# duckmayr/gpirt

Measured on AMD Instinct MI355X. Metric: MCMC iterations/sec at N=8192 x m=1024, higher is better.
Workload: dtype f64

## Files before the change

gpirt_amd/_lib.py:

```python
from __future__ import annotations

import ctypes as C
import os

import numpy as np

HERE = os.path.dirname(os.path.abspath(__file__))
LIB_PATH = os.environ.get("GPIRT_HIP_LIBRARY") or os.path.join(HERE, "libgpirt_hip.so")

NGRID = 1001
RNG_RSTREAM, RNG_ITEM = 0, 1
ST_INIT_F, ST_INIT_BETA, ST_F_Z, ST_F_ESS, ST_FSTAR, ST_THETA, ST_BETA = 1, 2, 3, 4, 5, 6, 7
ST_PPC = 8
ST_ELL = 9
ST_AMP = 10
ST_CARRY = 11

E_ARG, E_HIP, E_NODEVICE, E_ALLOC, E_RNG, E_INTERRUPT, E_NUMERIC = -1, -2, -3, -4, -5, -6, -7

SUM_THETA_BETA, SUM_F, SUM_PRED, SUM_WAIC = 1, 2, 4, 8
SUM_PARTS = {"theta_beta": SUM_THETA_BETA, "f": SUM_F, "pred": SUM_PRED, "waic": SUM_WAIC}
SUM_DIAG = 16
SUM_THETA_HIST, SUM_IRF_BAND = 32, 128
SUM_PARTS.update(diag=SUM_DIAG, theta_hist=SUM_THETA_HIST, irf_band=SUM_IRF_BAND)
# ... 670 lines not shown
    "gpirt_sampler_shape_order_state": (_i32, [_vp, C.POINTER(_vp), C.POINTER(_i64)]),
    "gpirt_shape_order_state_bytes": (_i32, [_i64, _i32, C.POINTER(_i64)]),
    "gpirt_shape_order_combine": (_i32, [_vp, _i32, C.POINTER(_vp), C.POINTER(ShapeOrder)]),
    "gpirt_sampler_summary_accumulate": (_i32, [_vp]),
    "gpirt_sampler_summary_get": (_i32, [_vp, C.c_char_p, _dp, _i64]),
    "gpirt_sampler_summary_totals": (_i32, [_vp, _dp]),
    "gpirt_sampler_create": (_i32, [C.POINTER(_vp), _vp, _dp, _i64, _i64, _dp, _dp, _dp, _dp,
                                     C.POINTER(Options), _vp]),
    "gpirt_sampler_destroy": (_i32, [_vp]),
    "gpirt_sampler_init": (_i32, [_vp]),
    "gpirt_sampler_step": (_i32, [_vp]),
    "gpirt_sampler_draw_f": (_i32, [_vp]),
    "gpirt_sampler_draw_fstar": (_i32, [_vp]),
    "gpirt_sampler_theta_partial": (_i32, [_vp]),
    "gpirt_sampler_theta_finish": (_i32, [_vp]),
    "gpirt_sampler_set_theta_block": (_i32, [_vp, _vp, _i64, _i64, _i64]),
    "gpirt_sampler_theta_block": (_i32, [_vp]),
    "gpirt_sampler_theta_commit": (_i32, [_vp]),
    "gpirt_sampler_draw_beta": (_i32, [_vp]),
    "gpirt_sampler_factor": (_i32, [_vp]),
    "gpirt_sampler_skip_factor": (_i32, [_vp]),
    "gpirt_sampler_adopt_factor": (_i32, [_vp, _i32]),
    "gpirt_sampler_build_cov": (_i32, [_vp]),
    "gpirt_sampler_panel_factor": (_i32, [_vp, _i64]),
    "gpirt_sampler_panel_update": (_i32, [_vp, _i64, _i64]),
    "gpirt_sampler_panel_copy": (_i32, [_vp, _i64, _vp, _i32]),
    "gpirt_sampler_panel_rows": (_i32, [_vp, C.POINTER(_i64)]),
    "gpirt_sampler_panel_factor_part": (_i32, [_vp, _i64, _i32]),
    "gpirt_sampler_panel_update_part": (_i32, [_vp, _i64, _i64, _i32]),
    "gpirt_sampler_panel_copy_part": (_i32, [_vp, _i64, _i32, _vp, _i64, _i32]),
    "gpirt_sampler_ldl": (_i32, [_vp, C.POINTER(_i64)]),
    "gpirt_sampler_nu_lr_draws": (_i32, [_vp, C.POINTER(_i64)]),
    "gpirt_sampler_ess_pack_draws": (_i32, [_vp, C.POINTER(_i64)]),
    "gpirt_sampler_nu_lr_rows": (_i32, [_vp, _vp, _i64]),
    "gpirt_sampler_fstar_free_draws": (_i32, [_vp, C.POINTER(_i64)]),
    "gpirt_sampler_factor_lr_count": (_i32, [_vp, C.POINTER(_i64)]),
    "gpirt_sampler_dense_factor_count": (_i32, [_vp, C.POINTER(_i64)]),
    "gpirt_sampler_dense_factor": (_i32, [_vp]),
    "gpirt_sampler_factor_lr_parts": (_i32, [_vp, _vp, _i64]),
    "gpirt_sampler_factor_lr_width": (_i32, [_vp, C.POINTER(_i32)]),
    "gpirt_sampler_factor_lr_blocks": (_i32, [_vp, _vp, _i64]),
    "gpirt_sampler_copy_state": (_i32, [_vp, _vp]),
    "gpirt_sampler_accumulate_irf": (_i32, [_vp]),
    "gpirt_sampler_iteration": (_i32, [_vp, C.POINTER(_i32)]),
    "gpirt_sampler_check": (_i32, [_vp]),
    "gpirt_sampler_devptr": (_i32, [_vp, C.c_char_p, C.POINTER(_vp), C.POINTER(_i64)]),
    "gpirt_sampler_get": (_i32, [_vp, C.c_char_p, _vp, _i64]),
    "gpirt_sampler_set": (_i32, [_vp, C.c_char_p, _dp, _i64]),
    "gpirt_sampler_finish_irfs": (_i32, [_vp, _i32, _dp]),
    "gpirt_sampler_enable_timing": (_i32, [_vp, _i32]),
    "gpirt_sampler_stage_times": (_i32, [_vp, _dp, _i32, C.POINTER(_i32), C.POINTER(C.c_char_p)]),
    "gpirt_prof_trailing": (_i32, [_vp, _i32, _dp, C.POINTER(_i64), _dp]),
    "gpirt_prof_enable": (_i32, [_vp, _i32]),
    "gpirt_prof_syrk": (_i32, [_vp, _i32, _i32, _dp, C.POINTER(_i64), _dp]),
    "gpirt_prof_syrk_bytes": (_i32, [_vp, _i32, _dp]),
    "gpirt_sampler_set_iteration": (_i32, [_vp, _i32]),
    "gpirt_ell_grid": (_i32, [_dbl, _dbl, _i32, _dp]),
    "gpirt_ell_check": (_i32, [_dbl, _dbl, _i32, _dp, _i32, _i32, C.POINTER(Kernel), C.POINTER(Options), _i64]),
    "gpirt_sampler_ell_enable": (_i32, [_vp, _dbl, _dbl, _i32, _dp, _i32, _i32, _i32]),
    "gpirt_sampler_draw_ell": (_i32, [_vp]),
    "gpirt_sampler_ell_width": (_i32, [_vp, _i32]),
    "gpirt_sampler_ell_get": (_i32, [_vp, C.c_char_p, _vp, _i64]),
    "gpirt_sampler_ell_stats": (_i32, [_vp, C.POINTER(Ell)]),
    "gpirt_sampler_draw_ell_centred": (_i32, [_vp]),
    "gpirt_sampler_ell_width_centred": (_i32, [_vp, _i32]),
    "gpirt_sampler_ell_centred_stats": (_i32, [_vp, C.POINTER(EllCentred)]),
# ... 109 lines not shown
```

gpirt_amd/csrc/api.hip:

```cpp
#include "common.h"
#include "kernels.h"
#include "rstream.h"

#include <stdarg.h>
#include <stdlib.h>
#include <new>
#include <vector>
#include <algorithm>

namespace gpirt {

static thread_local char g_err[512] = "";

static int env_value(const char* name, int dflt)
{
    const char* v = getenv(name);
    if (!v || !*v) return dflt;
    return atoi(v);
}
const Config& env_config()
{
    static const Config c = [] {
        Config d;
        d.nbo = env_value("GPIRT_NBO", d.nbo);            d.nbp = env_value("GPIRT_NBP", d.nbp);
        d.lookahead = env_value("GPIRT_LOOKAHEAD", d.lookahead);
        d.panel = env_value("GPIRT_PANEL", d.panel);      d.defer = env_value("GPIRT_DEFER", d.defer);
        d.trsm_inv = env_value("GPIRT_TRSM_INV", d.trsm_inv);
        d.ll_exact = env_value("GPIRT_LL_EXACT", d.ll_exact);
        d.ess_screen = env_value("GPIRT_ESS_SCREEN", d.ess_screen);
        d.theta_fixed = env_value("GPIRT_THETA_FIXED", d.theta_fixed);
        d.bordered = env_value("GPIRT_BORDERED", d.bordered);
        d.early_inv = env_value("GPIRT_EARLY_INV", d.early_inv);
        d.prep_early = env_value("GPIRT_PREP_EARLY", d.prep_early);
        d.guard_verbose = env_value("GPIRT_GUARD_VERBOSE", d.guard_verbose);
        d.rs_predict = env_value("GPIRT_RS_PREDICT", d.rs_predict);
        d.rs_lr = env_value("GPIRT_RS_LR", d.rs_lr);
        d.nu_lr = env_value("GPIRT_NU_LR", d.nu_lr);
        d.nu_sub = env_value("GPIRT_NU_SUB", NU_LR_SUB);
        d.fstar_free = env_value("GPIRT_FSTAR_FREE", d.fstar_free);
        d.factor_lr = env_value("GPIRT_FACTOR_LR", d.factor_lr);
        d.flr_fuse = env_value("GPIRT_FLR_FUSE", d.flr_fuse);
        d.flr_narrow = env_value("GPIRT_FLR_NARROW", d.flr_narrow);
        d.beta_screen = env_value("GPIRT_BETA_SCREEN", d.beta_screen);
        d.zfill_compact = env_value("GPIRT_ZFILL_COMPACT", d.zfill_compact);
        d.ess_pack = env_value("GPIRT_ESS_PACK", d.ess_pack);
        if (d.nbo < 64) d.nbo = 1024;
        if (d.nbp != 0 && d.nbp < 64) d.nbp = 512;
        return d;
    }();
    return c;
}

void set_error(const char* fmt, ...)
{
    va_list ap;
    va_start(ap, fmt);
    vsnprintf(g_err, sizeof(g_err), fmt, ap);
    va_end(ap);
}

int ensure_work(gpirt_handle_t h, size_t bytes)
{
    if (bytes <= h->work_bytes) return 0;
    GP_HIP(hipStreamSynchronize(h->stream));
    if (h->d_work) GP_HIP(hipFree(h->d_work));
    h->d_work = nullptr;
    h->work_bytes = 0;
    hipError_t e = hipMalloc(&h->d_work, bytes);
    if (e != hipSuccess) { set_error("hipMalloc(%zu) failed: %s", bytes, hipGetErrorString(e)); return GPIRT_E_ALLOC; }
    h->work_bytes = bytes;
    GP_HIP(poison_fresh(h, h->d_work, bytes, h->stream));
    return 0;
}

static int check_device(int device)
{
    int count = 0;
    hipError_t e = hipGetDeviceCount(&count);
// ... 55 lines not shown
}

}

using namespace gpirt;

static int create_own_stream(gpirt_handle_t* out, int device, bool high_priority);
namespace gpirt {
int create_side_handle(gpirt_handle_t* out, int device) { return create_own_stream(out, device, true); }
}

namespace gpirt {
int prof_pair_begin(gpirt_handle_t h, hipStream_t stream, ProfPair& pp)
{
    pp = ProfPair{nullptr, nullptr, 0.0, 0, 0.0};
    if (!h->prof.enabled) return 0;
    if (!h->prof.free_pairs.empty()) { pp = h->prof.free_pairs.back(); h->prof.free_pairs.pop_back(); }
    else { GP_HIP(hipEventCreate(&pp.e0)); GP_HIP(hipEventCreate(&pp.e1)); }
    GP_HIP(hipEventRecord(pp.e0, stream));
    return 0;
}
int prof_pair_end(gpirt_handle_t h, hipStream_t stream, ProfPair& pp, int cls, double flops, double bytes)
{
    if (!pp.e0) return 0;
    GP_HIP(hipEventRecord(pp.e1, stream));
    pp.flops = flops; pp.bytes = bytes; pp.cls = cls;
    h->prof.pending.push_back(pp);
    return 0;
}
}

extern "C" {

int gpirt_version(void) { return 143; }

const char* gpirt_last_error(void) { return g_err; }

int gpirt_device_count(int* count)
{
    GP_ARG(count != nullptr);
    int c = 0;
    hipError_t e = hipGetDeviceCount(&c);
    *count = (e == hipSuccess) ? c : 0;
    return 0;
}

int gpirt_create(gpirt_handle_t* out, int device, void* stream)
{
    GP_ARG(out != nullptr);
    *out = nullptr;
    GP_TRY(check_device(device < 0 ? 0 : device));
    if (device >= 0) GP_HIP(hipSetDevice(device));
    int cur = 0;
    GP_HIP(hipGetDevice(&cur));
    hipDeviceProp_t prop;
    GP_HIP(hipGetDeviceProperties(&prop, cur));
    if (strncmp(prop.gcnArchName, "gfx950", 6) != 0) {
        set_error("device %d is %s; libgpirt_hip is built for gfx950 (MI355X) only", cur, prop.gcnArchName);
        return GPIRT_E_NODEVICE;
    }
    gpirt_handle_s* h = new (std::nothrow) gpirt_handle_s();
    if (!h) { set_error("out of host memory"); return GPIRT_E_ALLOC; }
    h->device = cur;
    h->cfg = env_config();
    h->n_cu = prop.multiProcessorCount;
    h->stream = (hipStream_t)stream;
    h->own_stream = false;
// ... 63 lines not shown
    hipError_t e = hipSuccess;
    if (high_priority) e = hipDeviceGetStreamPriorityRange(&lo_pri, &hi_pri);
    if (e == hipSuccess)
        e = high_priority ? hipStreamCreateWithPriority(&st, hipStreamNonBlocking, hi_pri)
                          : hipStreamCreateWithFlags(&st, hipStreamNonBlocking);
    if (e != hipSuccess) { set_error("hipStreamCreate failed: %s", hipGetErrorString(e)); return GPIRT_E_HIP; }
    const int rc = gpirt_create(out, device, st);
    if (rc != 0) { hipStreamDestroy(st); return rc; }
    (*out)->own_stream = true;
    return 0;
}

int gpirt_create_own_stream(gpirt_handle_t* out, int device) { return create_own_stream(out, device, false); }

static int* config_slot(gpirt_handle_t h, const char* name, bool* read_only)
{
    struct E { const char* k; int* p; bool ro; } tab[] = {
        { "GPIRT_NBO", &h->cfg.nbo, true }, { "GPIRT_NBP", &h->cfg.nbp, true },
        { "GPIRT_LOOKAHEAD", &h->cfg.lookahead, false }, { "GPIRT_PANEL", &h->cfg.panel, false },
        { "GPIRT_DEFER", &h->cfg.defer, false }, { "GPIRT_TRSM_INV", &h->cfg.trsm_inv, false },
        { "GPIRT_LL_EXACT", &h->cfg.ll_exact, false }, { "GPIRT_ESS_SCREEN", &h->cfg.ess_screen, false }, { "GPIRT_THETA_FIXED", &h->cfg.theta_fixed, false }, { "GPIRT_BORDERED", &h->cfg.bordered, false },
        { "GPIRT_EARLY_INV", &h->cfg.early_inv, false }, { "GPIRT_PREP_EARLY", &h->cfg.prep_early, false },
        { "GPIRT_RS_PREDICT", &h->cfg.rs_predict, false },
        { "GPIRT_RS_LR", &h->cfg.rs_lr, false },
        { "GPIRT_NU_LR", &h->cfg.nu_lr, false },
        { "GPIRT_NU_SUB", &h->cfg.nu_sub, false },
        { "GPIRT_FSTAR_FREE", &h->cfg.fstar_free, false },
        { "GPIRT_FACTOR_LR", &h->cfg.factor_lr, false },
        { "GPIRT_FLR_FUSE", &h->cfg.flr_fuse, false },
        { "GPIRT_FLR_NARROW", &h->cfg.flr_narrow, false },
        { "GPIRT_BETA_SCREEN", &h->cfg.beta_screen, false },
        { "GPIRT_ZFILL_COMPACT", &h->cfg.zfill_compact, false },
        { "GPIRT_ESS_PACK", &h->cfg.ess_pack, false },
    };
    for (auto& e : tab)
        if (strcmp(e.k, name) == 0) { if (read_only) *read_only = e.ro; return e.p; }
    return nullptr;
}

int gpirt_config_get(gpirt_handle_t h, const char* name, int* value)
{
    GP_ARG(h && name && value);
    int* p = config_slot(h, name, nullptr);
    if (!p) { set_error("unknown switch '%s'", name); return GPIRT_E_ARG; }
    *value = *p;
    return 0;
}

int gpirt_config_set(gpirt_handle_t h, const char* name, int value)
{
    GP_ARG(h && name);
    bool ro = false;
    int* p = config_slot(h, name, &ro);
    if (!p) { set_error("unknown switch '%s'", name); return GPIRT_E_ARG; }
    if (ro) { set_error("%s is fixed per process (set it in the environment before the library is loaded)", name); return GPIRT_E_ARG; }
    if (p == &h->cfg.nu_sub && !nu_lr_sub_ok(value)) { set_error("GPIRT_NU_SUB must be 64, 128, 256 or 512 (got %d)", value); return GPIRT_E_ARG; }
    GP_HIP(hipStreamSynchronize(h->stream));
    *p = value;
    if (h->aux) *config_slot(h->aux, name, nullptr) = value;
    return 0;
}

void gpirt_kernel_default(gpirt_kernel* k)
{
    if (!k) return;
    memset(k, 0, sizeof(*k));
// ... 475 lines not shown
{
    GP_ARG(h && d_beta && d_theta && d_y && d_f && d_pm && d_ps && d_step && n >= 0 && m >= 0);
    BetaArgs a{};
    a.beta = d_beta; a.theta = d_theta; a.y = d_y; a.f = d_f; a.pm = d_pm; a.ps = d_ps; a.step = d_step;
    a.n = n; a.m = m; a.N = GPIRT_NGRID; a.mu = nullptr; a.mu_star = nullptr;
    a.seed = seed; a.iter = iter; a.item0 = 0; a.U = nullptr; a.path = d_path;
    if (h->cfg.beta_screen == 1 && n <= 8192 && n * m > 0) {
        GP_TRY(ensure_work(h, 8 * sizeof(double)));
        int* bad = reinterpret_cast<int*>(h->d_work);
        GP_HIP(hipMemsetAsync(bad, 0, sizeof(int), h->stream));
        GP_TRY(launch_check_y(h->stream, d_y, n * m, bad));
        GP_HIP(hipMemcpyAsync(h->h_info, bad, sizeof(int), hipMemcpyDeviceToHost, h->stream));
        GP_HIP(hipStreamSynchronize(h->stream));
        a.screen = *h->h_info == 0;
    }
    return launch_draw_beta(h->stream, a);
}

int gpirt_draw_beta(gpirt_handle_t h, double* d_beta, const double* d_theta, const double* d_y,
                    const double* d_f, const double* d_pm, const double* d_ps, const double* d_step,
                    int64_t n, int64_t m, uint64_t seed, uint32_t iter)
{
    return draw_beta_op(h, d_beta, d_theta, d_y, d_f, d_pm, d_ps, d_step, n, m, seed, iter, nullptr);
}

int gpirt_draw_beta_paths(gpirt_handle_t h, double* d_beta, const double* d_theta, const double* d_y,
                          const double* d_f, const double* d_pm, const double* d_ps, const double* d_step,
                          int64_t n, int64_t m, uint64_t seed, uint32_t iter, int* d_path)
{
    GP_ARG(d_path != nullptr);
    return draw_beta_op(h, d_beta, d_theta, d_y, d_f, d_pm, d_ps, d_step, n, m, seed, iter, d_path);
}

int gpirt_prof_enable(gpirt_handle_t h, int on)
{
    GP_ARG(h != nullptr);
    h->prof.enabled = on != 0;
    return 0;
}

static int prof_resolve(gpirt_handle_t h)
{
    if (h->prof.pending.empty()) return 0;
    GP_HIP(hipStreamSynchronize(h->stream));
    if (h->side) GP_HIP(hipStreamSynchronize(h->side));
    float longest4 = 0.f;
    {
        std::vector<float> d4;
        for (auto& pp : h->prof.pending)
            if (pp.cls == 4) { float ms = 0.f; GP_HIP(hipEventElapsedTime(&ms, pp.e0, pp.e1)); d4.push_back(ms); }
        if (!d4.empty()) { std::sort(d4.begin(), d4.end()); longest4 = d4[(d4.size() * 3) / 4]; }
    }
    for (auto& pp : h->prof.pending) {
        float ms = 0.f;
        GP_HIP(hipEventElapsedTime(&ms, pp.e0, pp.e1));
        if (pp.cls == 4 && ms < 0.25f * longest4) { h->prof.free_pairs.push_back(pp); continue; }
        h->prof.ms[pp.cls] += ms;
        h->prof.launches[pp.cls] += 1;
        h->prof.flops[pp.cls] += pp.flops;
        h->prof.bytes[pp.cls] += pp.bytes;
        h->prof.free_pairs.push_back(pp);
    }
    h->prof.pending.clear();
    return 0;
}

// ... 104 lines not shown
```

gpirt_amd/csrc/common.h:

```cpp
#pragma once

#include <hip/hip_runtime.h>
#include <stdint.h>
#include <stdio.h>
#include <string.h>
#include <math.h>
#include <vector>

#include "../../include/gpirt_hip.h"

namespace gpirt {

void set_error(const char* fmt, ...);

#define GP_HIP(call)                                                                         \
    do {                                                                                     \
        hipError_t e_ = (call);                                                              \
        if (e_ != hipSuccess) {                                                              \
            gpirt::set_error("%s failed: %s (%s:%d)", #call, hipGetErrorString(e_), __FILE__, \
                             __LINE__);                                                      \
            return GPIRT_E_HIP;                                                              \
        }                                                                                    \
    } while (0)

// ... 14 lines not shown
constexpr int PROF_CLASSES = 6;
struct ProfPair { hipEvent_t e0, e1; double flops; int cls; double bytes; };
struct Prof {
    bool        enabled = false;
    double      ms[PROF_CLASSES] = {};
    int64_t     launches[PROF_CLASSES] = {};
    double      flops[PROF_CLASSES] = {};
    double      bytes[PROF_CLASSES] = {};
    std::vector<ProfPair> pending;
    std::vector<ProfPair> free_pairs;
};

struct Config {
    int  nbo = 1024, nbp = 0;
    int  lookahead = 1;
    int  panel = 1;
    int  defer = 0;
    int  trsm_inv = 1;
    int  ll_exact = 0;
    int  theta_fixed = 1;
    int  ess_screen = 1;
    int  bordered = 1;
    int  early_inv = 1;
    int  prep_early = 1;
    int  rs_lr = 1;
    int  nu_lr = 1;
    int  nu_sub = 0;
    int  fstar_free = 1;
    int  factor_lr = 1;
    int  flr_fuse = 1;
    int  flr_narrow = 1;
    int  beta_screen = 1;
    int  ess_pack = 1;
    int  zfill_compact = 1;
    int  rs_predict = 1;
    int  guard_verbose = 0;
};
const Config& env_config();

struct KernelSpec {
    int    family = GPIRT_KERNEL_SE;
    double length_scale = 1.0;
    double inv_ell = 1.0;
    bool is_default() const { return family == GPIRT_KERNEL_SE && length_scale == 1.0; }
};

}

struct gpirt_handle_s {
    int          device = 0;
    gpirt::Config cfg;
    gpirt::KernelSpec kern;
    hipStream_t  stream = nullptr;
    bool         own_stream = false;
    int*         d_info = nullptr;
    int*         h_info = nullptr;
    double*      d_work = nullptr;
    size_t       work_bytes = 0;
    gpirt::Prof  prof;
    hipStream_t  side = nullptr;
    hipEvent_t   ev_fork = nullptr, ev_join = nullptr, ev_mid = nullptr, ev_half = nullptr;
    gpirt_handle_t aux = nullptr;
    const double* inv_partial_L = nullptr;
    int64_t      inv_partial_pairs = 0;
    bool         slim_leaf = false;
    hipEvent_t   ev_prelast = nullptr;
// ... 161 lines not shown
```

gpirt_amd/csrc/kernels.h:

```cpp
#pragma once

#include "common.h"

namespace gpirt {

enum { TRI_NONE = 0, TRI_SYRK_LOWER = 1, TRI_A_LOWER = 2, TRI_A_UPPER = 3, TRI_SYRK_LOWER_TRAILING = 4,
       TRI_SYRK_LOWER_BACKGROUND = 5  };
bool gemm_trailing_uses_128(int64_t M, int64_t N, bool background = false);
int launch_gemm_update_potf2(hipStream_t stream, int64_t M, int64_t N, int64_t K, const double* P, int64_t ldp,
                             double* C, int64_t ldc, int nb_next, int k0_next, int* info);

int launch_gemm(gpirt_handle_t h, hipStream_t stream, bool ta, bool tb, int tri, int64_t M,
                int64_t N, int64_t K, double alpha, const double* A, int64_t lda, const double* B,
                int64_t ldb, double beta, double* C, int64_t ldc, int64_t Mread = 0, const int* run_if = nullptr);

int launch_gemm_batched(hipStream_t stream, bool ta, bool tb, int tri, int64_t M, int64_t N, int64_t K, double alpha,
                        const double* A, int64_t lda, int64_t strideA, const double* B, int64_t ldb, int64_t strideB,
                        double beta, double* C, int64_t ldc, int64_t strideC, int batch);
int launch_gemm_batched_dual(hipStream_t stream, int tri, int64_t M, int64_t N, int64_t K, const double* A, int64_t lda,
                             int64_t strideA, const double* B, int64_t ldb, int64_t strideB, int64_t K2, const double* A2,
                             int64_t lda2, int64_t strideA2, const double* B2, int64_t ldb2, int64_t strideB2, double* C,
                             int64_t ldc, int64_t strideC, int batch);

int launch_syrk_panels(hipStream_t stream, int64_t M, int64_t N, int64_t kpart, int nparts, double alpha, const double* A,
// ... 380 lines not shown
struct TfDims { int64_t mp, ksteps, iblocks, gblocks; };
TfDims tf_dims(int64_t n, int64_t m, int64_t N);
size_t tf_y8_bytes(const TfDims& d);
size_t tf_gq_bytes(const TfDims& d);
size_t tf_aux_bytes(const TfDims& d);
int* tf_overflow(void* aux, const TfDims& d);
int launch_tf_indicators(hipStream_t stream, const double* y, int64_t n, int64_t ldy, int64_t m, const TfDims& d, void* Y8);
int launch_theta_fixed(hipStream_t stream, const double* fstar, int64_t N, int64_t n, int64_t m, const TfDims& d,
                       const void* Y8, void* Gq, void* aux, double* logpost, int64_t ldlp, bool trace = false,
                       gpirt_handle_t prof = nullptr);
long long* tf_trace(void* aux, const TfDims& d);
int tf_trace_wgs();
struct ThetaArgs {
    const double* logpost;
    int64_t N, n;
    int64_t i0;
    int stabilise;
    uint64_t seed; uint32_t iter;
    const double* U; uint64_t* pos; uint64_t cap;
    double* theta_out; int* degenerate; int* err;
    const double* log_prior; const int32_t* codes;
};
int launch_theta_sample(hipStream_t stream, const ThetaArgs& a);

struct BetaArgs {
    double* beta; const double* theta; const double* y; const double* f;
    const double* pm; const double* ps; const double* step;
    int64_t n, m, N;
    double* mu; double* mu_star;
    uint64_t seed; uint32_t iter; uint32_t item0;
    const double* U; uint64_t* pos; const uint64_t* item_off; uint64_t cap; int* err;
    int screen;
    int* path;
};
int launch_draw_beta(hipStream_t stream, const BetaArgs& a);
int launch_linear_mean(hipStream_t stream, const double* x, int64_t n, const double* beta, int64_t m, double* mu);

int prof_pair_begin(gpirt_handle_t h, hipStream_t stream, ProfPair& pp);
int prof_pair_end(gpirt_handle_t h, hipStream_t stream, ProfPair& pp, int cls, double flops, double bytes);

int report_panel_guard(gpirt_handle_t h, const int* info_words, hipStream_t stream);

int create_side_handle(gpirt_handle_t* out, int device);

constexpr int SUM_LAYOUT_VERSION = 1;
constexpr int SUM_HEADER_WORDS = 8;
struct SumLayout {
    int64_t tb_mean = -1, tb_m2 = -1, lse = -1, ll_mean = -1, ll_m2 = -1, y = -1, p_sum = -1, f_mean = -1, f_m2 = -1, irf = -1;
    int64_t dtb[7] = { -1, -1, -1, -1, -1, -1, -1 };
    int64_t df[7] = { -1, -1, -1, -1, -1, -1, -1 };
    int64_t total = 0;
};
enum { DG_H1_MEAN, DG_H1_M2, DG_H2_MEAN, DG_H2_M2, DG_BSUM, DG_BM_MEAN, DG_BM_M2 };
SumLayout summary_layout(int64_t n, int64_t m, int parts);
struct QntLayout {
    int64_t th_hist[3] = { -1, -1, -1 };
    int64_t th_off = -1;
    int64_t psum = -1;
    int64_t band_nan = -1;
    int64_t band = -1;
    int64_t total = 0;
};
QntLayout quantile_layout(int64_t n, int64_t m, int parts);
void irf_band_edges(double* out);
struct SummaryState {
    int parts = 0;
    int64_t n = 0, m = 0, draws = 0, planned = 0;
    double* block = nullptr;
// ... 521 lines not shown
```

gpirt_amd/csrc/sampler.hip:

```cpp
#include "common.h"
#include "kernels.h"
#include "rstream.h"

#include <stdlib.h>
#include <new>
#include <mutex>
#include <type_traits>
#include <string>
#include <vector>

using namespace gpirt;

namespace {

constexpr int KSPLIT = 16;

enum { ST_DRAW_F = 0, ST_FSTAR, ST_THETA_GEMM, ST_THETA_SAMPLE, ST_BETA, ST_FACTOR, ST_COUNT };
const char* const kStageNames[ST_COUNT] = { "draw_f", "draw_fstar", "theta_gemm", "theta_sample",
                                            "draw_beta", "factor" };

}

enum { ELL_WHITENED = 0, ELL_CENTRED = 1 };
struct EllUpdate {
// ... 88 lines not shown
    BetaCentredArgs a{};
    int prior_ok = -1;
    hipEvent_t tev[4] = {};
    double last_ms = 0.0, item_ms = 0.0;
};

struct ScaleState {
    bool on = false;
    uint32_t t[2] = {};
    double width[2] = {};
    ScaleArgs a{};
    int last_kind = -1;
    int prior_ok = -1;
    hipEvent_t tev[7] = {};
    double last_ms[2] = {};
    double times[6] = {};
};

struct CarryState {
    int64_t calls = 0;
    unsigned long long* counters = nullptr;
    double* quad = nullptr;
    hipEvent_t tev[2] = {};
    double last_ms = 0.0;
};

struct gpirt_sampler_s {
    gpirt_handle_t h = nullptr;
    int64_t n = 0, m = 0, N = GPIRT_NGRID;
    gpirt_options opt{};
    KernelSpec kern;
    RStream* rs = nullptr;
    double *y = nullptr, *Ypm = nullptr, *theta = nullptr, *theta_new = nullptr, *f = nullptr,
           *Z = nullptr, *NU = nullptr, *beta = nullptr, *mu = nullptr, *mu_star = nullptr,
           *fstar = nullptr, *L = nullptr, *tstar = nullptr, *kstar = nullptr, *rhs = nullptr,
           *mean = nullptr, *s = nullptr, *Gpm = nullptr, *logpost = nullptr, *irf_sum = nullptr,
           *pm = nullptr, *ps = nullptr, *step = nullptr;
    int kr = 0;
    double *knodes = nullptr, *kV = nullptr, *kparts = nullptr, *kP = nullptr;
    int64_t ext = 0, ldl = 0, node_off = -1, rank_off = 0;
    bool ext_grid = false, rows_valid = false, fstar_rows = false;
    double *nu_nodes = nullptr, *nu_wts = nullptr, *nuV = nullptr, *nuT = nullptr;
    bool nu_kern_ok = false, theta_ok = false, theta_alone = false;
    int64_t nu_lr_draws = 0;
    gpirt_handle_t haux = nullptr;
    hipEvent_t ev_trmm = nullptr, ev_prep = nullptr;
    bool prep_valid = false, prep_pending = false;
    double *ffF = nullptr, *ffW = nullptr;
    bool ff_have = false, prep_free = false;
    double ff_ell = 0.0;
    int64_t fstar_free_draws = 0;
    double *theta_L = nullptr, *flrG = nullptr, *flrXh = nullptr, *flrX = nullptr, *flrD = nullptr;
    bool L_structured = false;
    int L_part_width = 0;
    hipEvent_t ev_flr = nullptr;
    int64_t factor_lr_count = 0, dense_factor_count = 0;
    uint32_t z_filled_iter = 0;
    hipEvent_t ev_zfill = nullptr;
    bool beta_deferred = false, beta_pending = false;
    hipEvent_t ev_beta = nullptr;
    int64_t blk_i0 = 0, blk_n = 0, blk_m = 0;
    double *Ypm_blk = nullptr, *Gpm_full = nullptr, *logpost_blk = nullptr, *fstar_full = nullptr, *theta_stage = nullptr;
    TfDims tfd{}, tfd_blk{};
    double *tf_y8 = nullptr, *tf_gq = nullptr, *tf_aux = nullptr, *tf_y8_blk = nullptr, *tf_gq_blk = nullptr, *tf_aux_blk = nullptr;
    int *ess_k = nullptr, *flags = nullptr;
    int *fstar_off = nullptr;
    int *h_flags = nullptr;
// ... 31 lines not shown
    bool initialised = false;
    bool sticky_info = false;
    bool factor_fresh = false;
    bool counted = false;
    bool in_init = false;
    bool timing = false;
    hipEvent_t ev[ST_COUNT + 1] = {};
    double stage_ms[ST_COUNT] = {};
    std::vector<void*> allocs;
    std::vector<double> host_tmp;
    SummaryState sum;
    PpcState ppc;
    RankState rank;
    ShapeState shape;
    ScoreState score;
    SumscoreState sumscore;
    EquateState equate;
    LooState loo;
    AcfState acf;
    GroupsState groups;
    EllState ell;
    AmpState amp;
    OrdState ord;
    PopState pop;
    CarryState carry;
    SmoothF sf;
    BetaCentredState bc;
    ScaleState sc;
    bool lp_current = false;
    bool mu_linear = false;
    uint32_t* ess_ypk = nullptr;
    bool ess_ypk_valid = false;
    int64_t ess_pack_draws = 0;
};

namespace {

template <typename T>
int dalloc(gpirt_sampler_s* s, T** p, size_t count, bool numbers = true)
{
    void* q = nullptr;
    const size_t bytes = (count ? count : 1) * sizeof(T);
    hipError_t e = hipMalloc(&q, bytes);
    if (e != hipSuccess) {
        set_error("hipMalloc(%zu bytes) failed: %s", bytes, hipGetErrorString(e));
        return GPIRT_E_ALLOC;
    }
    s->allocs.push_back(q);
    *p = reinterpret_cast<T*>(q);
    if (std::is_same<T, double>::value || std::is_same<T, float>::value) {
        if (numbers && poison_fresh(s->h, q, bytes, s->h->stream) != hipSuccess) {
            set_error("hipMemsetAsync(%zu bytes) failed", bytes);
            return GPIRT_E_HIP;
        }
    }
    return 0;
}

inline bool stream_mode(const gpirt_sampler_s* s) { return s->opt.rng_kind == GPIRT_RNG_RSTREAM; }

int report_degenerate_theta(gpirt_sampler_s* s, int count);

void ahead_generate(gpirt_sampler_s* s, uint32_t* dst, uint64_t count)
{
    constexpr uint64_t EVERY = 1ull << 16;
    while (count) {
        const uint64_t c = count < EVERY ? count : EVERY;
        s->snaps.emplace_back(s->ahead_gen, *s->rs);
        s->rs->fill_raw(dst, c);
        s->ahead_gen += c; dst += c; count -= c;
    }
}

void ahead_resolve(void* owner, bool gone)
{
    gpirt_sampler_s* s = static_cast<gpirt_sampler_s*>(owner);
    if (s->ahead_attached) {
        if (s->ev_up) hipEventSynchronize(s->ev_up);
        size_t best = 0;
        for (size_t q = 0; q < s->snaps.size(); ++q) if (s->snaps[q].first <= s->ahead_used) best = q;
        *s->rs = s->snaps[best].second;
        s->rs->skip(s->ahead_used - s->snaps[best].first);
    }
    s->ahead_attached = false;
    s->snaps.clear();
    s->ahead_gen = s->ahead_used = s->a_len = 0;
    if (s->rs_obj) { s->rs_obj->owner = nullptr; s->rs_obj->resolve = nullptr; }
    if (gone) { s->rs_obj = nullptr; s->rs = nullptr; }
}

void rstream_forget(void* sampler)
{
// ... 223 lines not shown
        if (nu_lr && s->prep_pending && s->prep_free) {
            GP_HIP(hipStreamWaitEvent(st, s->ev_prep, 0));
            s->prep_pending = false;
        }
        if (s->z_filled_iter == iter && s->ev_zfill) {
            GP_HIP(hipStreamWaitEvent(st, s->ev_zfill, 0));
            s->z_filled_iter = 0;
        } else {
            GP_TRY(z_sync(s));
            GP_TRY(launch_item_uniforms(st, s->opt.seed, iter, GPIRT_ST_F_Z, (uint32_t)s->opt.item0, m, n, s->Z, true, s->h->cfg.zfill_compact == 1));
        }
        {
            ProfPair pp;
            GP_TRY(prof_pair_begin(h, st, pp));
            if (nu_lr) {
                double flops = 0.0, bytes = 0.0;
                NuLrArgs q{};
                q.L = s->L; q.ldl = s->ldl; q.Bt = s->L + n + s->node_off; q.V = s->nuV; q.Z = s->Z; q.NU = s->NU; q.T = s->nuT;
                q.n = n; q.m = m; q.sub = h->cfg.nu_sub;
                GP_TRY(launch_nu_lr_basis(st, s->theta, n, s->nu_nodes, s->nu_wts, s->nuV));
                if (free) GP_HIP(hipEventRecord(s->ev_trmm, st));
                GP_TRY(launch_nu_lr(st, q, &flops, &bytes));
                GP_TRY(prof_pair_end(h, st, pp, 3, flops, bytes));
                s->nu_lr_draws += 1;
            } else {
                GP_TRY(launch_gemm(h, st, false, false, TRI_A_LOWER, n, m, n, 1.0, s->L, s->ldl, s->Z, n, 0.0, s->NU, n));
                GP_TRY(prof_pair_end(h, st, pp, 3, (double)n * (double)n * (double)m, 8.0 * (0.5 * (double)n * (double)n + 2.0 * (double)n * (double)m)));
            }
        }
        if (s->amp.mode) GP_TRY(launch_amp_scale(st, s->NU, s->amp.amp, n, m));
        if (prep && !early && !free) GP_HIP(hipEventRecord(s->ev_trmm, st));
        if (s->ord.on) {
            EssOrdArgs a{};
            a.f = s->f; a.nu = s->NU; a.mu = s->mu; a.cat = s->ord.cat; a.thr = s->ord.thr; a.counts = s->ord.counts;
            a.C = s->ord.C; a.n = n; a.m = m; a.k_out = s->ess_k; a.err = s->flags;
            a.seed = s->opt.seed; a.iter = iter; a.item0 = (uint32_t)s->opt.item0;
            a.screen = h->cfg.ess_screen == 1;
            GP_TRY(launch_ess_ord(st, a));
        } else {
        EssArgs a{};
        a.f = s->f; a.nu = s->NU; a.y = s->y; a.mu = s->mu; a.n = n; a.m = m; a.k_out = s->ess_k;
        a.err = s->flags; a.seed = s->opt.seed; a.iter = iter; a.item0 = (uint32_t)s->opt.item0;
        a.ll_exact = h->cfg.ll_exact;
        a.screen = h->cfg.ess_screen == 1;
        if (h->cfg.ess_pack != 2 && s->mu_linear && s->ess_ypk && !s->opt.kernel_fp32 && ess_pack_eligible(n)) {
            if (!s->ess_ypk_valid) { GP_TRY(launch_ess_pack(st, s->y, n, m, s->ess_ypk)); s->ess_ypk_valid = true; }
            a.ypk = s->ess_ypk; a.theta = s->theta; a.beta = s->beta;
            a.grid = h->cfg.ess_pack == 3 ? 2 * h->n_cu : 0;
            s->ess_pack_draws += 1;
        }
        GP_TRY(launch_ess(st, a));
        }
        if (prep) {
            hipStream_t ax = s->haux->stream;
            GP_HIP(hipStreamWaitEvent(ax, s->ev_trmm, 0));
            if (free) {
                GP_TRY(fstar_prep_free(s, ax, !nu_lr));
            } else {
                s->haux->slim_leaf = early;
                const int rc_prep = fstar_prep(s, s->haux);
                s->haux->slim_leaf = false;
                GP_TRY(rc_prep);
            }
            GP_HIP(hipEventRecord(s->ev_prep, ax));
            s->prep_valid = true; s->prep_pending = true; s->prep_free = free;
        }
        return 0;
    }
    auto plain_item = [&](int64_t j) -> int {
        GP_TRY(launch_rstream_normals(st, s->U, s->pos, 0, n, 1, s->Z));
        GP_TRY(launch_trmv_lower(st, s->L, n, s->ldl, s->Z, s->NU + n, s->NU));
        EssArgs a{};
        a.f = s->f + j * n; a.nu = s->NU; a.y = s->y + j * n; a.mu = s->mu + j * n; a.n = n; a.m = 1;
        a.k_out = s->ess_k + j; a.err = s->flags; a.item0 = (uint32_t)j;
        a.U = s->U; a.pos = s->pos; a.cap = s->U_cap;
        return launch_ess(st, a);
    };
    const bool spec = s->spec_ok;
    if (!spec) {
        for (int64_t j = 0; j < m; ++j) GP_TRY(plain_item(j));
        return 0;
    }
    bool tiles64 = false;
    Rs3Args a{};
    a.U = s->U; a.cap = s->U_cap; a.Nrm = s->Nrm; a.anchor = s->anchor; a.pos = s->pos; a.posv = s->posv; a.k_out = s->ess_k;
    a.err = s->flags; a.n = n; a.m = m; a.Lt = s->Lt; a.nkb = rs_tile_quads(n); a.part = s->rs_part;
    a.units = s->rs_units; a.nunits = s->rs_nunits; a.nfull = s->rs_nfull;
    a.lim1 = RS3_C1; a.lim2 = RS3_C2;
    if (h->rs_cand_limit > 0) {
        if (h->rs_cand_limit < a.lim1) a.lim1 = h->rs_cand_limit;
        if (h->rs_cand_limit < a.lim2) a.lim2 = h->rs_cand_limit;
    }
    a.f = s->f; a.y = s->y; a.mu = s->mu; a.partial = s->rs_partial; a.flags = s->rs_flags;
    GP_TRY(launch_rs3_begin(st, a, (uint64_t)m * (2ull * (uint64_t)n + 2ull) + 512ull * (uint64_t)m + 4096ull));
    int64_t pass = 0, done = 0;
    int64_t one_phase = 0;
    bool topped = false;
    bool predict = h->cfg.rs_predict != 2;
    bool lr = predict && s->lr_on, lr_missed = false;
    bool tiles32_full = !lr;
    if (predict) GP_TRY(launch_rs32_tiles(st, s->L, n, s->ldl, s->Lt32, lr));
    if (lr) {
        RsLrSetup q{};
        q.theta = s->theta; q.n = n; q.nodes = s->lr_nodes; q.wts = s->lr_wts; q.Mn = s->lr_M; q.eps = GPIRT_JITTER; q.L = s->L; q.ldl = s->ldl;
        q.V64 = s->lr_V64; q.Gb = s->lr_Gb; q.V32t = s->lr_V32t; q.Ct32 = s->lr_Ct32; q.nk8 = rs32_tile_octs(n); q.bad = s->lr_bad;
        GP_TRY(launch_rs_lr_setup(st, q));
    }
    while (done < m) {
        const int64_t left = m - done;
        int64_t count = (left + RS3_SLOTS - 1) / RS3_SLOTS + left / 40 + 2;
        if (one_phase > 4 * m + 64) { set_error("R-stream replay: draw_f made no progress"); return GPIRT_E_NUMERIC; }
        if (predict) {
            count = (left + RS3_SLOTS - 1) / RS3_SLOTS + left / 8 + 4;
            if (s->rs_pass_rate > 0.0) {
                const int64_t hint = (int64_t)(s->rs_pass_rate * 1.03 * (double)left) + 4;
                if (hint < count) count = hint;
            }
            Rs3Args ap = a;
            ap.anchor = s->anchorP; ap.pos = s->rs_posP; ap.k_out = s->rs_kpred; ap.err = s->rs_errP;
            ap.units = s->rs_unitsP; ap.nunits = s->rs_nunitsP; ap.nfull = s->rs_nfullP;
            if (!lr && !tiles32_full) { GP_TRY(launch_rs32_tiles(st, s->L, n, s->ldl, s->Lt32)); tiles32_full = true; }
            ap.lr = lr ? 1 : 0;
            if (lr) {
                ap.units = s->lr_units; ap.nunits = ap.nfull = s->lr_nunits;
                ap.Ct32 = s->lr_Ct32; ap.lrY = s->lr_Y; ap.V32t = s->lr_V32t;
            }
            ap.Lt32 = s->Lt32; ap.nk8 = rs32_tile_octs(n); ap.part32 = s->rs_part32; ap.mispredict = h->rs_mispredict;
            ap.dec_part = s->rs_dec_part; ap.dec_rec = s->rs_dec_rec; ap.dec_ticket = s->rs_dec_ticket; ap.pass_count = s->rs_ctl + 3;
            GP_TRY(launch_rs_pred_start(st, s->anchor, s->anchorP, s->ess_k, m));
            for (int64_t q = 0; q < count; ++q, ++pass) {
                s->rs_tag += 1ull << 20;
                ap.tag = s->rs_tag;
                ap.trace = (h->rs_trace_pass >= 0 && pass == h->rs_trace_pass) ? s->rs_trace : nullptr;
                ProfPair pp;
                GP_TRY(prof_pair_begin(h, st, pp));
                GP_TRY(launch_rs3p_products(st, ap));
                const double pass_el = lr ? (double)(RS3P_KC + RS_LR_RANK) * (double)n : 0.5 * (double)n * (double)(n + 1);
                GP_TRY(prof_pair_end(h, st, pp, 4, 2.0 * RS3_CAND * pass_el, 4.0 * pass_el));
                if (lr) GP_TRY(launch_rs_lr_apply(st, ap));
                GP_TRY(launch_rs3p_decide(st, ap));
            }
            const int64_t mc = m - done;
            GP_TRY(launch_rs_gather(st, s->Nrm, s->posv, s->anchorP, n, done, m, s->Z));
            GP_TRY(launch_gemm(h, st, false, false, TRI_A_LOWER, n, mc, n, 1.0, s->L, s->ldl, s->Z, n, 0.0, s->NU, n));
            RsVerifyArgs v{};
            v.f = s->f; v.nu = s->NU; v.y = s->y; v.mu = s->mu; v.n = n; v.m = m; v.j0 = done;
            v.U = s->U; v.cap = s->U_cap; v.posv = s->posv; v.anchorP = s->anchorP;
            v.kv = s->rs_kv; v.used = s->rs_used; v.ierr = s->rs_ierr;
            GP_TRY(launch_rs_verify(st, v));
            GP_TRY(launch_rs_commit(st, v, s->anchor, s->pos, s->rs_ctl, s->flags, s->f, s->ess_k));
        } else {
        if (!tiles64) { GP_TRY(launch_rs_tiles(st, s->L, n, s->ldl, s->Lt)); tiles64 = true; }
        for (int64_t q = 0; q < count; ++q, ++pass, ++one_phase) {
            s->rs_tag += 1ull << 20;
            a.tag = s->rs_tag;
            a.trace = (h->rs_trace_pass >= 0 && pass == h->rs_trace_pass) ? s->rs_trace : nullptr;
            ProfPair pp;
            GP_TRY(prof_pair_begin(h, st, pp));
            GP_TRY(launch_rs3_products(st, a));
            GP_TRY(prof_pair_end(h, st, pp, 4, 2.0 * RS3_CAND * 0.5 * (double)n * (double)(n + 1), 8.0 * 0.5 * (double)n * (double)(n + 1)));
            GP_TRY(launch_rs3_slice(st, a));
        }
        }
        GP_HIP(hipMemcpyAsync(s->h_next, s->anchor, sizeof(uint64_t), hipMemcpyDeviceToHost, st));
        GP_HIP(hipMemcpyAsync(s->h_next + 1, s->flags, sizeof(int), hipMemcpyDeviceToHost, st));
        if (predict) GP_HIP(hipMemcpyAsync(s->h_next + 2, s->rs_ctl + 3, sizeof(uint64_t), hipMemcpyDeviceToHost, st));
        if (predict) GP_HIP(hipMemcpyAsync(s->h_next + 3, s->rs_ctl + 1, sizeof(uint64_t), hipMemcpyDeviceToHost, st));
        if (lr) GP_HIP(hipMemcpyAsync(s->h_next + 4, s->lr_bad, sizeof(int), hipMemcpyDeviceToHost, st));
        if (s->stream_open && !topped) { GP_TRY(ahead_topup(s, stream_window(s))); topped = true; }
        GP_HIP(hipStreamSynchronize(st));
        if ((int)s->h_next[1] != 0) break;
        if (predict) {
            if (lr && (int)s->h_next[4] != 0) { s->lr_on = false; lr = false; }
            if (lr && s->h_next[3] != s->rs_mis_seen) { lr = false; lr_missed = true; }
            s->rs_mis_seen = s->h_next[3];
        }
        if ((int64_t)s->h_next[0] <= done) {
            if (predict) {
                predict = false;
// ... 164 lines not shown
    s->lp_current = false;
    s->mu_linear = false;
    s->theta_ok = true;
    return 0;
}

int do_theta_block(gpirt_sampler_s* s)
{
    hipStream_t st = s->h->stream;
    const int64_t N = s->N, nb = s->blk_n, mt = s->blk_m;
    const int64_t Np = (N + 127) / 128 * 128;
    GP_HIP(hipMemsetAsync(s->theta_stage, 0, sizeof(double) * (size_t)s->n, st));
    if (nb == 0) return 0;
    const int* only_if = nullptr;
    if (s->h->cfg.theta_fixed == 1) {
        GP_TRY(launch_theta_fixed(st, s->fstar_full, N, nb, mt, s->tfd_blk, s->tf_y8_blk, s->tf_gq_blk, s->tf_aux_blk, s->logpost_blk, N, false, s->h));
        only_if = tf_overflow(s->tf_aux_blk, s->tfd_blk);
    }
    GP_TRY(launch_loglik_terms(st, s->fstar_full, N, mt, s->Gpm_full, Np, only_if));
    GP_TRY(launch_gemm(s->h, st, false, true, TRI_NONE, N, nb, 2 * mt, 1.0, s->Gpm_full, Np, s->Ypm_blk, nb, 0.0,
                       s->logpost_blk, N, Np, only_if));
    GP_TRY(launch_theta_nan_fix(st, s->Gpm_full, Np, s->Ypm_blk, nb, mt, s->logpost_blk, N, N, only_if));
    ThetaArgs a{};
    a.logpost = s->logpost_blk; a.N = N; a.n = nb; a.i0 = s->blk_i0; a.stabilise = s->opt.theta_stabilise;
    a.seed = s->opt.seed; a.iter = (uint32_t)(s->iter + 1);
    a.theta_out = s->theta_stage; a.degenerate = s->flags + 1; a.err = s->flags;
    return launch_theta_sample(st, a);
}

int launch_beta_on(gpirt_sampler_s* s, hipStream_t st)
{
    s->lp_current = false;
    s->mu_linear = !s->ord.on;
    if (s->ord.on) {
        BetaOrdArgs a{};
        a.beta = s->beta; a.theta = s->theta; a.cat = s->ord.cat; a.f = s->f; a.thr = s->ord.thr; a.pm = s->pm; a.ps = s->ps;
        a.step = s->step; a.C = s->ord.C; a.n = s->n; a.m = s->m; a.N = s->N; a.mu = s->mu; a.mu_star = s->mu_star;
        a.seed = s->opt.seed; a.iter = (uint32_t)(s->iter + 1); a.item0 = (uint32_t)s->opt.item0;
        return launch_draw_beta_ord(st, a);
    }
    BetaArgs a{};
    a.beta = s->beta; a.theta = s->theta; a.y = s->y; a.f = s->f; a.pm = s->pm; a.ps = s->ps;
    a.step = s->step; a.n = s->n; a.m = s->m; a.N = s->N; a.mu = s->mu; a.mu_star = s->mu_star;
    a.seed = s->opt.seed; a.iter = (uint32_t)(s->iter + 1); a.item0 = (uint32_t)s->opt.item0;
    a.err = s->flags;
    a.screen = s->h->cfg.beta_screen == 1;
    if (stream_mode(s)) { a.U = s->U; a.pos = s->pos; a.item_off = s->beta_off; a.cap = s->U_cap; }
    GP_TRY(launch_draw_beta(st, a));
    if (stream_mode(s)) GP_TRY(launch_advance_pos(st, s->pos, s->beta_total));
    return 0;
}

int beta_sync(gpirt_sampler_s* s)
{
    if (s->beta_deferred) {
        s->beta_deferred = false;
        GP_TRY(launch_beta_on(s, s->h->stream));
    }
    if (s->beta_pending) {
        GP_HIP(hipStreamWaitEvent(s->h->stream, s->ev_beta, 0));
        s->beta_pending = false;
    }
    return 0;
}

int do_draw_beta(gpirt_sampler_s* s)
{
    const bool defer = s->h->cfg.early_inv != 2 && !stream_mode(s) && s->haux && s->ev_beta && s->initialised;
    GP_TRY(beta_sync(s));
    if (defer) { s->beta_deferred = true; return 0; }
    return launch_beta_on(s, s->h->stream);
}

int carry_refusals(gpirt_sampler_s* s, int nugget, const char* entry)
{
    if (!s->initialised) { set_error("%s needs an initialised sampler (gpirt_sampler_init)", entry); return GPIRT_E_ARG; }
    if (stream_mode(s)) {
        set_error("carry: rng = reference (GPIRT_RNG_RSTREAM) is refused, R's stream has no such draw");
        return GPIRT_E_ARG;
    }
// ... 325 lines not shown
    int j = (int)floor(u0 * (double)(2 * w));
    if (j > 2 * w - 1) j = 2 * w - 1;
    const int kp = e.k + (j < w ? j - w : j - w + 1);
    if (kp < 0 || kp >= e.P) { counted(); c.last_proposed = kp; c.out_of_range += 1; c.last = 2; return 0; }
    GP_TRY(ell_join(s));
    GP_TRY(ensure_dense_factor(s));
    s->factor_fresh = false;
    const bool timed = s->timing;
    if (timed)
        for (hipEvent_t& t : e.tev) if (!t) GP_HIP(hipEventCreate(&t));
    auto tick = [&](int i) { if (timed) hipEventRecord(e.tev[i], st); };
    const KernelSpec kern_before = s->kern;
    const bool rows_before = s->rows_valid;
    const size_t fbytes = sizeof(double) * (size_t)(n * m), lbytes = sizeof(double) * (size_t)(s->ldl * n);
    auto restore = [&]() -> int {
        s->kern = kern_before;
        s->rows_valid = rows_before;
        invalidate_factor_products(s);
        GP_HIP(hipMemcpyAsync(s->L, e.Lsave, lbytes, hipMemcpyDeviceToDevice, st));
        return 0;
    };
    tick(0);
    GP_HIP(hipMemcpyAsync(s->NU, s->f, fbytes, hipMemcpyDeviceToDevice, st));
    if (kind == ELL_CENTRED) GP_HIP(hipMemcpyAsync(e.nuprop, s->f, fbytes, hipMemcpyDeviceToDevice, st));
    GP_HIP(hipMemcpyAsync(e.Lsave, s->L, lbytes, hipMemcpyDeviceToDevice, st));
    tick(1);
    GP_TRY(launch_trsm_lower(h, st, s->L, n, s->ldl, s->NU, m, n, false));
    tick(2);
    ell_set_kernel(s, e.grid[(size_t)kp]);
    int rc = factor_core(s);
    c.factorisations += 1;
    tick(3);
    const double lp_diff = e.log_prior[(size_t)kp] - e.log_prior[(size_t)e.k], log_u = log(u1);
    for (int attempt = 0; !rc; ++attempt) {
        if (kind == ELL_WHITENED) {
            rc = launch_gemm(h, st, false, false, TRI_A_LOWER, n, m, n, 1.0, s->L, s->ldl, s->NU, n, 0.0, e.fprop, n);
            tick(4);
            if (!rc) rc = launch_ell_delta(st, s->f, e.fprop, s->mu, s->y, n, m, e.delta, e.nonfin);
            tick(5);
            if (!rc) rc = launch_ell_decide(st, e.delta, e.nonfin, m, lp_diff, log_u, h->d_info, e.rec, e.flag);
            tick(6);
            if (!rc) rc = launch_ell_commit(st, e.flag, s->f, e.fprop, n * m);
            tick(7);
        } else {
            if (attempt > 0 && hipMemcpyAsync(e.nuprop, s->f, fbytes, hipMemcpyDeviceToDevice, st) != hipSuccess) {
                set_error("length-scale update: copying f failed: %s", hipGetErrorString(hipGetLastError()));
                rc = GPIRT_E_HIP;
            }
            if (!rc) rc = launch_trsm_lower(h, st, s->L, n, s->ldl, e.nuprop, m, n, false);
            tick(4);
            if (!rc) rc = launch_ell_quad(st, s->NU, e.nuprop, n, m, e.dq, e.nonfin);
            tick(5);
            if (!rc) rc = launch_ell_logdet(st, e.Lsave, s->L, n, s->ldl, e.ld);
            tick(6);
            if (!rc) rc = launch_ell_decide_centred(st, e.dq, e.nonfin, m, e.ld, lp_diff, log_u, h->d_info, e.rec_c, e.flag);
            tick(7);
        }
        if (rc) break;
        if (hipMemcpyAsync(e.h_flag, e.flag, sizeof(int), hipMemcpyDeviceToHost, st) != hipSuccess ||
            hipStreamSynchronize(st) != hipSuccess) {
            set_error("length-scale update: reading the decision failed: %s", hipGetErrorString(hipGetLastError()));
            rc = GPIRT_E_HIP;
            break;
        }
        if (*e.h_flag != 3) break;
        if (attempt > 0 || h->cfg.panel == 2) {
            hipMemcpyAsync(h->h_info, h->d_info, 8 * sizeof(int), hipMemcpyDeviceToHost, st);
            hipStreamSynchronize(st);
            rc = report_panel_guard(h, h->h_info, st);
            break;
        }
// ... 160 lines not shown
{
    GP_ARG(s && d_state && bytes);
    const Block<St> b = of(s);
    GP_TRY(needs(b));
    if (seal) GP_TRY(seal(s->h->stream, b.st));
    else GP_HIP(hipStreamSynchronize(s->h->stream));
    *d_state = b.block;
    *bytes = words(b.st) * (int64_t)sizeof(uint64_t);
    return 0;
}

template <class St>
int stage_get(gpirt_sampler_t s, BlockOf<St> of, int (*get)(hipStream_t, St*, const char*, void*, int64_t), const char* name,
              void* h_out, int64_t bytes)
{
    GP_ARG(s && name && h_out && bytes >= 0);
    const Block<St> b = of(s);
    GP_TRY(needs(b));
    return get(s->h->stream, b.st, name, h_out, bytes);
}

template <class St, class Alloc>
int stage_enable(gpirt_sampler_t s, St* st, void (*release)(St*), bool on, Alloc alloc)
{
    GP_HIP(hipStreamSynchronize(s->h->stream));
    release(st);
    if (!on) return 0;
    const int rc = alloc();
    if (rc) release(st);
    return rc;
}

struct DrawView { const double *theta, *beta, *f, *mu, *fstar, *gbar; uint32_t iter; };
DrawView live_view(gpirt_sampler_t s) { return { s->theta, s->beta, s->f, s->mu, s->fstar, s->shape.gbar, (uint32_t)s->iter }; }

int acc_summary(gpirt_sampler_t s, const DrawView& v) { return launch_summary_accumulate(s->h->stream, &s->sum, v.theta, v.beta, v.f, v.mu, s->y, v.fstar); }
int acc_ppc(gpirt_sampler_t s, const DrawView& v) { return launch_ppc_accumulate(s->h->stream, &s->ppc, v.f, v.mu, s->y, s->opt.seed, v.iter, v.theta); }
int acc_rank(gpirt_sampler_t s, const DrawView& v) { return launch_rank_accumulate(s->h->stream, &s->rank, v.theta); }
int acc_score(gpirt_sampler_t s, const DrawView& v) { return launch_score_accumulate(s->h, s->h->stream, &s->score, v.fstar); }
int acc_shape(gpirt_sampler_t s, const DrawView& v) { return launch_shape_accumulate(s->h->stream, &s->shape, v.gbar); }
int acc_sumscore(gpirt_sampler_t s, const DrawView& v) { return launch_sumscore_accumulate(s->h->stream, &s->sumscore, v.fstar); }
int acc_equate(gpirt_sampler_t s, const DrawView& v) { return launch_equate_accumulate(s->h, s->h->stream, &s->equate, v.fstar); }
int acc_loo(gpirt_sampler_t s, const DrawView& v) { return launch_loo_accumulate(s->h->stream, &s->loo, v.f, v.mu); }
int acc_acf(gpirt_sampler_t s, const DrawView& v) { return launch_acf_accumulate(s->h->stream, &s->acf, v.theta, v.beta, v.f, v.mu, s->y); }
int acc_groups(gpirt_sampler_t s, const DrawView& v) { return launch_groups_accumulate(s->h->stream, &s->groups, v.theta, v.f, v.mu, s->y); }

int accumulate_run(gpirt_sampler_t s, const DrawView& v)
{
    if (s->sum.parts) GP_TRY(acc_summary(s, v));
    if (s->ppc.on) GP_TRY(acc_ppc(s, v));
    if (s->rank.on) GP_TRY(acc_rank(s, v));
    if (s->score.on) GP_TRY(acc_score(s, v));
    if (s->shape.on) GP_TRY(acc_shape(s, v));
    if (s->sumscore.on) GP_TRY(acc_sumscore(s, v));
    if (s->equate.on) GP_TRY(acc_equate(s, v));
    if (s->loo.on) GP_TRY(acc_loo(s, v));
    return 0;
}

template <class St>
int stage_accumulate(gpirt_sampler_t s, BlockOf<St> of, int (*piece)(gpirt_sampler_t, const DrawView&), bool join_beta = false)
{
    GP_ARG(s && s->initialised);
    GP_TRY(needs(of(s)));
    if (join_beta) GP_TRY(beta_sync(s));
    return piece(s, live_view(s));
}

int check_top(const char* what, int top, int max)
{
    if (top >= 1 && top <= max) return 0;
    set_error("%s: top = %d is outside 1..%d", what, top, max);
    return GPIRT_E_ARG;
}

int score_check_new(const double* h_y_new, int64_t n_new, int64_t m)
{
    for (int64_t g = 0; g < n_new * m; ++g) {
// ... 50 lines not shown
    int rc = 0;
#define GP_A(p, cnt) do { rc = dalloc(s, &(p), (size_t)(cnt)); if (rc) { gpirt_sampler_destroy(s); return rc; } } while (0)
    GP_A(s->y, n * m);       GP_A(s->Ypm, n * 2 * m);  GP_A(s->theta, n);       GP_A(s->theta_new, n);
    s->tfd = tf_dims(n, m, N);
#define GP_AI(p, cnt) do { rc = dalloc(s, &(p), (size_t)(cnt), false); if (rc) { gpirt_sampler_destroy(s); return rc; } } while (0)
    GP_AI(s->tf_y8, tf_y8_bytes(s->tfd) / 8 + 2); GP_AI(s->tf_gq, tf_gq_bytes(s->tfd) / 8 + 2); GP_AI(s->tf_aux, tf_aux_bytes(s->tfd) / 8 + 2);
#undef GP_AI
    GP_A(s->f, n * m);       GP_A(s->Z, n * m);        GP_A(s->NU, n * (m > 1 + TRMV_SPLIT ? m : 1 + TRMV_SPLIT));   GP_A(s->beta, 2 * m);
    s->kr = s->opt.kstar_rank;
    if (s->kr != 0 && (!s->opt.fstar_fused || s->kr < 16 || s->kr > 128 || (s->kr % 16) != 0)) {
        set_error("kstar_rank must be a multiple of 16 in 16..128 and needs fstar_fused");
        gpirt_sampler_destroy(s);
        return GPIRT_E_ARG;
    }
    if (s->opt.factor_structured != 0 && s->opt.factor_structured != 1) {
        set_error("factor_structured must be 0 or 1");
        gpirt_sampler_destroy(s);
        return GPIRT_E_ARG;
    }
    const bool bordered_ok = (n % 64) == 0 && h->cfg.bordered != 2;
    if (bordered_ok) {
        if (s->kr == NU_LR_RANK) { s->ext = s->kr; s->node_off = 0; s->rank_off = 0; s->fstar_rows = true; }
        else if (s->kr > 0) { s->ext = NU_LR_RANK + s->kr; s->node_off = 0; s->rank_off = NU_LR_RANK; s->fstar_rows = true; }
        else if (n >= 1024) {
            s->node_off = (N + 63) / 64 * 64;
            s->ext = s->node_off + NU_LR_RANK;
            s->ext_grid = true; s->fstar_rows = true;
        } else { s->ext = NU_LR_RANK; s->node_off = 0; }
    } else if ((n % 64) == 0) { s->ext = NU_LR_RANK; s->node_off = 0; }
    s->ldl = n + s->ext;
    s->theta_ok = true;
    for (int64_t i = 0; i < n; ++i) s->theta_ok = s->theta_ok && h_theta0[i] >= -5.0 && h_theta0[i] <= 5.0;
    s->nu_kern_ok = nu_kernel_ok(s->kern);
    GP_A(s->mu, n * m);      GP_A(s->mu_star, N * m + 1); GP_A(s->fstar, N * m + 1); GP_A(s->L, s->ldl * n);
    GP_A(s->tstar, N + 1);   GP_A(s->rhs, n * (N + m) + 2); GP_A(s->mean, N * m + 1); GP_A(s->s, N + 1);
    GP_A(s->Gpm, ((N + 127) / 128 * 128) * 2 * m + 2); GP_A(s->logpost, N * n + 2); GP_A(s->irf_sum, N * m + 1);
    if (hipMemsetAsync(s->Gpm, 0, sizeof(double) * (size_t)(((N + 127) / 128 * 128) * 2 * m + 2), st) != hipSuccess) {
        set_error("hipMemsetAsync(Gpm) failed"); gpirt_sampler_destroy(s); return GPIRT_E_HIP;
    }
    GP_A(s->pm, 2 * m);      GP_A(s->ps, 2 * m);       GP_A(s->step, 2 * m);
    GP_A(s->ess_k, m);       GP_A(s->flags, 4);
    if (!stream_mode(s) && ess_pack_eligible(n)) {
        rc = dalloc(s, &s->ess_ypk, (size_t)(512 * m), false);
        if (rc) { gpirt_sampler_destroy(s); return rc; }
    }
    if (!s->opt.fstar_fused) GP_A(s->kstar, n * N + 2);
    if (s->node_off >= 0) {
        GP_A(s->nu_nodes, NU_LR_RANK); GP_A(s->nu_wts, NU_LR_RANK);
        if (!stream_mode(s)) {
            GP_A(s->nuV, n * NU_LR_RANK); GP_A(s->nuT, nu_lr_slabs(n) * NU_LR_RANK * m);
            if (hipMemsetAsync(s->nuT, 0, sizeof(double) * (size_t)(NU_LR_RANK * m), st) != hipSuccess) {
                set_error("hipMemsetAsync(nuT) failed"); gpirt_sampler_destroy(s); return GPIRT_E_HIP;
            }
        }
        if (!stream_mode(s) && s->kr == NU_LR_RANK && s->fstar_rows) {
            GP_A(s->ffF, FSTAR_FREE_RANK * FSTAR_FREE_RANK); GP_A(s->ffW, 2 * FSTAR_FREE_RANK * FSTAR_FREE_RANK);
            if (s->opt.factor_structured) {
                const int64_t fp = factor_lr_parts(n, NU_LR_SUB_MIN) * NU_LR_RANK * NU_LR_RANK;
                GP_A(s->theta_L, n); GP_A(s->flrG, fp); GP_A(s->flrXh, fp); GP_A(s->flrX, NU_LR_RANK * n);
                GP_A(s->flrD, factor_lr_parts(n) * (NU_LR_PART / 64) * NU_LR_RANK * NU_LR_RANK);
            }
        }
    }
    if (s->kr != 0) {
        GP_A(s->knodes, s->kr); GP_A(s->kV, N * s->kr);
        GP_A(s->kparts, (size_t)KSPLIT * s->kr * (s->kr + m)); GP_A(s->kP, (size_t)s->kr * (s->kr + m));
    }
    if (stream_mode(s)) {
        std::vector<uint64_t> off((size_t)m);
        uint64_t acc = 0;
        for (int64_t j = 0; j < m; ++j) {
            off[(size_t)j] = acc;
            for (int k = 0; k < 2; ++k) {
                const double sd = h_step[k + 2 * j];
                acc += ((sd > 0.0 && std::isfinite(sd)) ? 2 : 0) + 1;
            }
        }
        s->beta_total = acc;
// ... 80 lines not shown
    if (hipHostMalloc(&s->h_flags, 4 * sizeof(int), hipHostMallocDefault) != hipSuccess) {
        set_error("pinned allocation failed"); gpirt_sampler_destroy(s); return GPIRT_E_ALLOC;
    }
    for (int i = 0; i <= ST_COUNT; ++i) hipEventCreate(&s->ev[i]);
    std::vector<double> ts((size_t)N);
    for (int64_t i = 0; i < N; ++i) ts[(size_t)i] = -5.0 + (double)i * 0.01;
    hipMemcpyAsync(s->y, h_y, sizeof(double) * (size_t)(n * m), hipMemcpyHostToDevice, st);
    hipMemcpyAsync(s->theta, h_theta0, sizeof(double) * (size_t)n, hipMemcpyHostToDevice, st);
    hipMemcpyAsync(s->pm, h_pm, sizeof(double) * (size_t)(2 * m), hipMemcpyHostToDevice, st);
    hipMemcpyAsync(s->ps, h_ps, sizeof(double) * (size_t)(2 * m), hipMemcpyHostToDevice, st);
    hipMemcpyAsync(s->step, h_step, sizeof(double) * (size_t)(2 * m), hipMemcpyHostToDevice, st);
    hipMemcpyAsync(s->tstar, ts.data(), sizeof(double) * (size_t)N, hipMemcpyHostToDevice, st);
    std::vector<double> nodes, V;
    if (s->kr > 0) {
        const int r = s->kr;
        cheb_nodes_basis(r, nodes, V);
        hipMemcpyAsync(s->knodes, nodes.data(), sizeof(double) * (size_t)r, hipMemcpyHostToDevice, st);
        hipMemcpyAsync(s->kV, V.data(), sizeof(double) * (size_t)(N * r), hipMemcpyHostToDevice, st);
    }
    if (s->node_off >= 0) {
        std::vector<double> nnodes, wts;
        nu_lr_nodes(nnodes, wts);
        hipMemcpyAsync(s->nu_nodes, nnodes.data(), sizeof(double) * NU_LR_RANK, hipMemcpyHostToDevice, st);
        hipMemcpyAsync(s->nu_wts, wts.data(), sizeof(double) * NU_LR_RANK, hipMemcpyHostToDevice, st);
        hipStreamSynchronize(st);
    }
    hipMemsetAsync(s->L, 0, sizeof(double) * (size_t)(s->ldl * n), st);
    hipMemsetAsync(s->irf_sum, 0, sizeof(double) * (size_t)(N * m), st);
    hipMemsetAsync(s->flags, 0, 4 * sizeof(int), st);
    hipMemsetAsync(s->ess_k, 0, sizeof(int) * (size_t)m, st);
    launch_indicators(st, s->y, n, m, s->Ypm);
    launch_tf_indicators(st, s->y, n, n, m, s->tfd, s->tf_y8);
    if (s->ess_ypk) { launch_ess_pack(st, s->y, n, m, s->ess_ypk); s->ess_ypk_valid = true; }
    if (hipStreamSynchronize(st) != hipSuccess || hipGetLastError() != hipSuccess) {
        set_error("sampler upload failed"); gpirt_sampler_destroy(s); return GPIRT_E_HIP;
    }
    if (fstar_free_setup(s) != 0) { gpirt_sampler_destroy(s); return GPIRT_E_HIP; }
    if (!stream_mode(s)) {
        if (!h->aux) {
            if (create_side_handle(&h->aux, h->device) != 0) { gpirt_sampler_destroy(s); return GPIRT_E_HIP; }
            h->aux->cfg = h->cfg;
        }
        s->haux = h->aux;
        s->haux->poison_allocs = h->poison_allocs;
        if (
            hipEventCreateWithFlags(&s->ev_trmm, hipEventDisableTiming) != hipSuccess ||
            hipEventCreateWithFlags(&s->ev_prep, hipEventDisableTiming) != hipSuccess ||
            hipEventCreateWithFlags(&s->ev_zfill, hipEventDisableTiming) != hipSuccess ||
            hipEventCreateWithFlags(&s->ev_flr, hipEventDisableTiming) != hipSuccess ||
            hipEventCreateWithFlags(&s->ev_beta, hipEventDisableTiming) != hipSuccess) {
            gpirt_sampler_destroy(s);
            return GPIRT_E_HIP;
        }
    }
    s->host_tmp.assign(h_pm, h_pm + 2 * m);
    s->host_tmp.insert(s->host_tmp.end(), h_ps, h_ps + 2 * m);
    h->live_samplers += 1;
    s->counted = true;
    *out = s;
    return 0;
}

int gpirt_sampler_destroy(gpirt_sampler_t s)
{
    if (!s) return 0;
    if (s->h) hipStreamSynchronize(s->h->stream);
// ... 82 lines not shown
                                                            (uint32_t)(s->opt.item0 + j), (uint32_t)p));
                b[(size_t)(p + 2 * j)] = v;
            }
        GP_HIP(hipMemcpyAsync(s->beta, b.data(), sizeof(double) * b.size(), hipMemcpyHostToDevice, st));
        GP_HIP(hipStreamSynchronize(st));
    } else {
        const uint64_t nf = (uint64_t)m * 2 * (uint64_t)n;
        s->saved = *s->rs;
        s->rs->fill_unif(s->hU, nf);
        std::vector<double> b((size_t)(2 * m));
        const double* pm = s->host_tmp.data();
        const double* ps = pm + 2 * m;
        uint64_t nb = 0;
        for (int64_t j = 0; j < m; ++j)
            for (int p = 0; p < 2; ++p) {
                const double mu = pm[p + 2 * j], sd = ps[p + 2 * j];
                double v;
                if (mu != mu || !std::isfinite(sd) || sd < 0.0) v = NAN;
                else if (sd == 0.0 || !std::isfinite(mu)) v = mu;
                else { v = mu + sd * s->rs->norm(); nb += 2; }
                b[(size_t)(p + 2 * j)] = v;
            }
        const uint64_t nfs = 2 * (uint64_t)N * (uint64_t)m;
        s->rs->fill_unif(s->hU + nf, nfs);
        (void)nb;
        GP_HIP(hipMemcpyAsync(s->U, s->hU, (nf + nfs) * sizeof(double), hipMemcpyHostToDevice, st));
        GP_HIP(hipMemsetAsync(s->pos, 0, sizeof(uint64_t), st));
        GP_TRY(launch_rstream_normals(st, s->U, s->pos, 2 * n, n, m, s->Z));
        GP_TRY(launch_gemm(h, st, false, false, TRI_A_LOWER, n, m, n, 1.0, s->L, s->ldl, s->Z, n, 0.0, s->f, n));
        GP_TRY(launch_advance_pos(st, s->pos, nf));
        GP_HIP(hipMemcpyAsync(s->beta, b.data(), sizeof(double) * b.size(), hipMemcpyHostToDevice, st));
        GP_HIP(hipStreamSynchronize(st));
    }
    GP_TRY(launch_linear_mean(st, s->theta, n, s->beta, m, s->mu));
    s->mu_linear = true;
    GP_TRY(launch_linear_mean(st, s->tstar, N, s->beta, m, s->mu_star));
    GP_TRY(do_draw_fstar(s, 0));
    if (stream_mode(s)) {
        GP_HIP(hipMemcpyAsync(s->h_pos, s->pos, sizeof(uint64_t), hipMemcpyDeviceToHost, st));
        GP_HIP(hipStreamSynchronize(st));
        const uint64_t nf = (uint64_t)m * 2 * (uint64_t)n;
        const uint64_t used_fstar = *s->h_pos - nf;
        RStream r = s->saved;
        r.skip(nf);
        const double* pm = s->host_tmp.data();
        const double* ps = pm + 2 * m;
        for (int64_t j = 0; j < m; ++j)
            for (int p = 0; p < 2; ++p) {
                const double mu = pm[p + 2 * j], sd = ps[p + 2 * j];
                if (!(mu != mu || !std::isfinite(sd) || sd < 0.0) && !(sd == 0.0 || !std::isfinite(mu))) {
                    (void)r.next32(); (void)r.next32();
                }
            }
        r.skip(used_fstar);
        *s->rs = r;
    }
    s->iter = 0;
    s->initialised = true;
    return 0;
}

int gpirt_sampler_draw_f(gpirt_sampler_t s) { GP_ARG(s && s->initialised); return do_draw_f(s); }
int gpirt_sampler_draw_fstar(gpirt_sampler_t s) { GP_ARG(s && s->initialised); return do_draw_fstar(s, (uint32_t)(s->iter + 1)); }
int gpirt_sampler_theta_partial(gpirt_sampler_t s) { GP_ARG(s && s->initialised); return do_theta_partial(s); }
int gpirt_sampler_theta_finish(gpirt_sampler_t s) { GP_ARG(s && s->initialised); return do_theta_finish(s); }

int gpirt_sampler_set_theta_block(gpirt_sampler_t s, const double* y_block, int64_t i0, int64_t n_block, int64_t m_total)
// ... 1067 lines not shown
    for (int k = 0; k < P; ++k) {
        const long double l = logl((long double)A.grid[(size_t)k]);
        A.log_prior[(size_t)k] = log_prior ? log_prior[k] : (double)(-(l * l) / 2.0L);
    }
    const int near1 = amp_nearest_one(A.grid.data(), P);
    std::vector<int> idx((size_t)m), wd((size_t)m, width);
    std::vector<double> amp((size_t)m);
    for (int64_t j = 0; j < m; ++j) {
        idx[(size_t)j] = k0 ? k0[j] : near1;
        amp[(size_t)j] = A.grid[(size_t)idx[(size_t)j]];
    }
    if (hipMemcpyAsync(A.d_grid, A.grid.data(), sizeof(double) * (size_t)P, hipMemcpyHostToDevice, st) != hipSuccess ||
        hipMemcpyAsync(A.d_log_prior, A.log_prior.data(), sizeof(double) * (size_t)P, hipMemcpyHostToDevice, st) != hipSuccess ||
        hipMemcpyAsync(A.amp, amp.data(), sizeof(double) * (size_t)m, hipMemcpyHostToDevice, st) != hipSuccess ||
        hipMemcpyAsync(A.idx, idx.data(), sizeof(int) * (size_t)m, hipMemcpyHostToDevice, st) != hipSuccess ||
        hipMemcpyAsync(A.width, wd.data(), sizeof(int) * (size_t)m, hipMemcpyHostToDevice, st) != hipSuccess ||
        hipMemsetAsync(A.rec, 0, sizeof(double) * 5 * (size_t)m, st) != hipSuccess ||
        hipMemsetAsync(A.counts, 0, sizeof(long long) * 4 * (size_t)m, st) != hipSuccess ||
        hipMemsetAsync(A.hist, 0, hist_bytes, st) != hipSuccess ||
        hipMemsetAsync(A.draws, 0, draw_bytes, st) != hipSuccess ||
        hipStreamSynchronize(st) != hipSuccess) return fail(GPIRT_E_HIP, "the upload");
    A.mode = 2;
    return 0;
}

int gpirt_sampler_draw_amp(gpirt_sampler_t s)
{
    GP_ARG(s && s->initialised);
    GP_TRY(ord_refuse(s, "gpirt_sampler_draw_amp", ORD_BINARY));
    AmpState& A = s->amp;
    GP_TRY(needs(A.mode == 2, "the amplitude update is", "gpirt_sampler_amp_enable"));
    GP_TRY(beta_sync(s));
    AmpUpdateArgs a{};
    a.f = s->f; a.mu = s->mu; a.y = s->y; a.n = s->n; a.m = s->m;
    a.grid = A.d_grid; a.log_prior = A.d_log_prior; a.P = A.P;
    a.idx = A.idx; a.width = A.width; a.amp = A.amp; a.counts = A.counts; a.rec = A.rec;
    a.seed = s->opt.seed; a.t = A.t + 1; a.item0 = (uint32_t)s->opt.item0;
    hipStream_t st = s->h->stream;
    const bool timed = s->timing;
    if (timed) {
        for (hipEvent_t& t : A.tev) if (!t) GP_HIP(hipEventCreate(&t));
        GP_HIP(hipEventRecord(A.tev[0], st));
    }
    GP_TRY(launch_amp_update(st, a));
    A.t += 1;
    if (timed) {
        GP_HIP(hipEventRecord(A.tev[1], st));
        GP_HIP(hipEventSynchronize(A.tev[1]));
        float ms = 0.f;
        hipEventElapsedTime(&ms, A.tev[0], A.tev[1]);
        A.last_ms = ms;
    }
    return 0;
}

int gpirt_sampler_amp_width(gpirt_sampler_t s, const int* w)
{
    GP_ARG(s && w);
    AmpState& A = s->amp;
    GP_TRY(needs(A.mode == 2, "the amplitude update is", "gpirt_sampler_amp_enable"));
    for (int64_t j = 0; j < s->m; ++j)
        if (w[j] < 1 || w[j] > A.P - 1) {
            set_error("amplitude: width[%lld] = %d, it must lie in 1 .. P - 1 = %d", (long long)j, w[j], A.P - 1);
            return GPIRT_E_ARG;
        }
    GP_HIP(hipMemcpyAsync(A.width, w, sizeof(int) * (size_t)s->m, hipMemcpyHostToDevice, s->h->stream));
    GP_HIP(hipStreamSynchronize(s->h->stream));
// ... 179 lines not shown
    if (s->opt.kernel_fp32) { set_error("%s: kernel_fp32 is refused, the single-precision build is the default kernel's alone", me); return GPIRT_E_ARG; }
    if (s->opt.item0 != 0 || (s->opt.m_total > 0 && s->opt.m_total != s->m)) {
        set_error("%s: an item shard (item0 = %lld, m_total = %lld) is refused, the amplitudes are kept for all items of one sampler", me,
                  (long long)s->opt.item0, (long long)s->opt.m_total);
        return GPIRT_E_ARG;
    }
    AmpState& A = s->amp;
    if (A.mode != 2) {
        set_error("%s: the amplitudes are not in the sampled mode (gpirt_sampler_amp_enable): %s", me,
                  A.mode == 1 ? "they are fixed" : "they are off");
        return GPIRT_E_ARG;
    }
    if (!s->nu_kern_ok) {
        if (s->kern.family != GPIRT_KERNEL_SE) {
            set_error("%s: the handle's kernel is not a squared exponential, it has no rank-64 form (gpirt_kernel_check(kernel, 64))", me);
            return GPIRT_E_ARG;
        }
        const int rc = kernel_rank_check(s->kern, AMP_CENTRED_RANK, nullptr, nullptr);
        if (rc) return rc;
        set_error("%s: the length-scale grid's smallest value fails gpirt_kernel_check(kernel, 64)", me);
        return GPIRT_E_ARG;
    }
    if (!s->theta_ok) {
        set_error("%s: a theta is not finite or lies outside [-5, 5], the rank-64 basis does not hold there", me);
        return GPIRT_E_ARG;
    }
    GP_TRY(beta_sync(s));
    s->lp_current = false;
    s->mu_linear = false;
    GP_TRY(amp_centred_alloc(s));
    GP_TRY(smooth_factor(s));
    AmpCentredArgs a = A.ca;
    a.F = s->sf.F; a.live = s->sf.live; a.r = s->sf.r;
    a.f = s->f; a.mu = s->mu; a.y = s->y; a.n = s->n; a.m = s->m;
    a.theta = s->theta; a.eps = GPIRT_JITTER;
    a.H = s->NU;
    a.grid = A.d_grid; a.log_prior = A.d_log_prior; a.P = A.P;
    a.idx = A.idx; a.amp = A.amp;
    a.seed = s->opt.seed; a.t = A.ct + 1; a.item0 = (uint32_t)s->opt.item0;
    a.err = s->flags;
    hipStream_t st = s->h->stream;
    const bool timed = s->timing;
    if (timed) {
        for (hipEvent_t& t : A.ctev) if (!t) GP_HIP(hipEventCreate(&t));
        GP_HIP(hipEventRecord(A.ctev[0], st));
    }
    GP_TRY(launch_amp_centred(st, a));
    A.ct += 1;
    if (timed) {
        GP_HIP(hipEventRecord(A.ctev[1], st));
        GP_HIP(hipEventSynchronize(A.ctev[1]));
        float ms = 0.f;
        hipEventElapsedTime(&ms, A.ctev[0], A.ctev[1]);
        A.clast_ms = ms;
    }
    return 0;
}

int gpirt_sampler_amp_centred_stats(gpirt_sampler_t s, gpirt_amp_centred* out)
{
    GP_ARG(s && out);
    const AmpState& A = s->amp;
    memset(out, 0, sizeof(*out));
    out->calls = A.ct; out->accept_rate = (double)NAN; out->last_ms = A.clast_ms;
    if (A.mode != 2 || !A.cbuf) return 0;
    out->rank = s->sf.have ? s->sf.r : 0;
    const int64_t m = s->m;
// ... 60 lines not shown
        return GPIRT_E_ARG;
    }
    if (!s->nu_kern_ok) {
        if (s->kern.family != GPIRT_KERNEL_SE) {
            set_error("%s: the handle's kernel is not a squared exponential, it has no rank-64 form (gpirt_kernel_check(kernel, 64))", me);
            return GPIRT_E_ARG;
        }
        const int rc = kernel_rank_check(s->kern, BETA_CENTRED_RANK, nullptr, nullptr);
        if (rc) return rc;
        set_error("%s: the length-scale grid's smallest value fails gpirt_kernel_check(kernel, 64)", me);
        return GPIRT_E_ARG;
    }
    if (!s->theta_ok) {
        set_error("%s: a theta is not finite or lies outside [-5, 5], the rank-64 basis does not hold there", me);
        return GPIRT_E_ARG;
    }
    BetaCentredState& Bc = s->bc;
    if (Bc.prior_ok < 0) {
        Bc.prior_ok = 1;
        const double* ps = s->host_tmp.data() + 2 * s->m;
        for (int64_t e = 0; e < 2 * s->m; ++e)
            if (!(ps[e] > 0.0) || !(ps[e] <= 1.79769313486231570815e308)) Bc.prior_ok = 0;
    }
    if (!Bc.prior_ok) {
        set_error("%s: a prior sd of beta is not finite and > 0, the conditional has no precision to add", me);
        return GPIRT_E_ARG;
    }
    GP_TRY(beta_sync(s));
    s->lp_current = false;
    s->mu_linear = false;
    GP_TRY(beta_centred_alloc(s));
    GP_TRY(smooth_factor(s));
    BetaCentredArgs a = Bc.a;
    a.f = s->f; a.beta = s->beta; a.mu = s->mu; a.mu_star = s->mu_star; a.n = s->n; a.m = s->m; a.N = s->N;
    a.theta = s->theta; a.tstar = s->tstar; a.pm = s->pm; a.ps = s->ps;
    a.amp = s->amp.mode ? s->amp.amp : nullptr;
    a.F = s->sf.F; a.eps = GPIRT_JITTER;
    a.seed = s->opt.seed; a.t = Bc.t + 1; a.item0 = (uint32_t)s->opt.item0;
    a.err = s->flags;
    hipStream_t st = s->h->stream;
    const bool timed = s->timing;
    if (timed) {
        for (hipEvent_t& t : Bc.tev) if (!t) GP_HIP(hipEventCreate(&t));
        GP_HIP(hipEventRecord(Bc.tev[0], st));
        a.kev[0] = Bc.tev[2]; a.kev[1] = Bc.tev[3];
    }
    GP_TRY(launch_beta_centred(st, a));
    Bc.t += 1;
    if (timed) {
        GP_HIP(hipEventRecord(Bc.tev[1], st));
        GP_HIP(hipEventSynchronize(Bc.tev[1]));
        float ms = 0.f;
        hipEventElapsedTime(&ms, Bc.tev[0], Bc.tev[1]);
        Bc.last_ms = ms;
        hipEventElapsedTime(&ms, Bc.tev[2], Bc.tev[3]);
        Bc.item_ms = ms;
    }
    return 0;
}

int gpirt_sampler_beta_centred_get(gpirt_sampler_t s, const char* name, void* h_out, int64_t bytes)
{
    GP_ARG(s && name && h_out);
    BetaCentredState& Bc = s->bc;
    if (strcmp(name, "time") == 0 || strcmp(name, "time_item") == 0) {
        if (bytes != 8) { set_error("beta (centred): '%s' holds 8 bytes, %lld were asked for", name, (long long)bytes); return GPIRT_E_ARG; }
        memcpy(h_out, name[4] ? &Bc.item_ms : &Bc.last_ms, 8);
// ... 108 lines not shown
        GP_HIP(hipMemsetAsync(a.bad, 0, sizeof(int) * n, st));
        GP_HIP(hipMemsetAsync(a.counts, 0, sizeof(long long) * 6, st));
        Sc.on = true;
    }
    Sc.width[0] = w_scale; Sc.width[1] = w_shift;
    return 0;
}

int gpirt_sampler_scale_width(gpirt_sampler_t s, int kind, double w)
{
    GP_ARG(s != nullptr);
    const char* me = "gpirt_sampler_scale_width";
    GP_TRY(needs(s->sc.on, "the scale and shift move is", "gpirt_sampler_scale_enable"));
    if (kind != 0 && kind != 1) { set_error("%s: kind = %d, it must be 0 (scale) or 1 (shift)", me, kind); return GPIRT_E_ARG; }
    GP_TRY(scale_width_check(me, kind, w));
    s->sc.width[kind] = w;
    return 0;
}

static int do_draw_scale(gpirt_sampler_t s, int kind, const char* me, bool timed)
{
    if (!s->initialised) { set_error("%s needs an initialised sampler (gpirt_sampler_init)", me); return GPIRT_E_ARG; }
    GP_TRY(needs(s->sc.on, "the scale and shift move is", "gpirt_sampler_scale_enable"));
    GP_TRY(scale_refusals(s, me));
    if (kind != 0 && kind != 1) { set_error("%s: kind = %d, it must be 0 (scale) or 1 (shift)", me, kind); return GPIRT_E_ARG; }
    GP_TRY(beta_sync(s));
    if (!s->lp_current) {
        set_error("%s: logpost is not current, the move belongs between gpirt_sampler_theta_partial and gpirt_sampler_theta_finish "
                  "(a stage that writes fstar, beta, f, theta or the population prior ran since the last theta_partial)", me);
        return GPIRT_E_ARG;
    }
    ScaleState& Sc = s->sc;
    ScaleArgs a = Sc.a;
    a.beta = s->beta; a.mu = s->mu; a.mu_star = s->mu_star; a.fstar = s->fstar; a.logpost = s->logpost;
    a.gbar = s->shape.on ? s->shape.gbar : nullptr;
    a.n = s->n; a.m = s->m; a.N = s->N; a.theta = s->theta; a.pm = s->pm; a.ps = s->ps;
    if (s->pop.mode) { a.log_prior = s->pop.log_prior; a.codes = s->pop.codes; }
    a.kind = kind; a.width = Sc.width[kind]; a.seed = s->opt.seed; a.t = Sc.t[kind] + 1;
    hipStream_t st = s->h->stream;
    if (timed) {
        for (hipEvent_t& t : Sc.tev) if (!t) GP_HIP(hipEventCreate(&t));
        GP_HIP(hipEventRecord(Sc.tev[0], st));
        for (int k = 0; k < 4; ++k) a.kev[k] = Sc.tev[3 + k];
    }
    s->mu_linear = false;
    GP_TRY(launch_scale_curve(st, a));
    if (timed) GP_HIP(hipEventRecord(Sc.tev[1], st));
    GP_TRY(theta_product(s, a.fstar2, a.logpost2));
    if (timed) GP_HIP(hipEventRecord(Sc.tev[2], st));
    GP_TRY(launch_scale_decide(st, a));
    Sc.t[kind] += 1;
    Sc.last_kind = kind;
    return 0;
}

static int scale_read_times(gpirt_sampler_t s)
{
    ScaleState& Sc = s->sc;
    GP_HIP(hipEventSynchronize(Sc.tev[6]));
    float ms = 0.f;
    hipEventElapsedTime(&ms, Sc.tev[0], Sc.tev[6]); Sc.times[0] = ms;
    hipEventElapsedTime(&ms, Sc.tev[0], Sc.tev[1]); Sc.times[1] = ms;
    hipEventElapsedTime(&ms, Sc.tev[1], Sc.tev[2]); Sc.times[2] = ms;
    for (int k = 0; k < 3; ++k) { hipEventElapsedTime(&ms, Sc.tev[3 + k], Sc.tev[4 + k]); Sc.times[3 + k] = ms; }
    Sc.last_ms[Sc.last_kind] = Sc.times[0];
    return 0;
}
// ... 406 lines not shown
        hipMalloc((void**)&A.hist, sizeof(uint32_t) * rows * Ps) != hipSuccess ||
        hipMalloc((void**)&A.draws, draw_bytes) != hipSuccess) return fail(GPIRT_E_ALLOC, "hipMalloc");
    A.C = C; A.P = P; A.W = W; A.lp_W = W; A.hi = hi; A.planned = planned_draws; A.recorded = 0; A.irf_draws = 0;
    A.grid.resize(Ps); A.log_prior.resize(Ps);
    ord_grid_fill(hi, P, A.grid.data());
    for (int k = 0; k < P; ++k) A.log_prior[(size_t)k] = log_prior ? log_prior[k] : -(A.grid[(size_t)k] * A.grid[(size_t)k]) / 18.0;
    std::vector<int> idx(rows);
    std::vector<double> thr(rows);
    for (int64_t j = 0; j < m; ++j)
        for (int c = 1; c < C; ++c) {
            const size_t r = (size_t)j * (size_t)(C - 1) + (size_t)(c - 1);
            idx[r] = K0 ? K0[r] : (2 * (P - 1) * c + C) / (2 * C);
            thr[r] = A.grid[(size_t)idx[r]];
        }
    if (hipMemcpyAsync(A.cat, cat, (size_t)(n * m), hipMemcpyHostToDevice, st) != hipSuccess ||
        hipMemcpyAsync(A.d_grid, A.grid.data(), sizeof(double) * Ps, hipMemcpyHostToDevice, st) != hipSuccess ||
        hipMemcpyAsync(A.d_log_prior, A.log_prior.data(), sizeof(double) * Ps, hipMemcpyHostToDevice, st) != hipSuccess ||
        hipMemcpyAsync(A.idx, idx.data(), sizeof(int) * rows, hipMemcpyHostToDevice, st) != hipSuccess ||
        hipMemcpyAsync(A.thr, thr.data(), sizeof(double) * rows, hipMemcpyHostToDevice, st) != hipSuccess ||
        hipMemsetAsync(A.lp, 0, sizeof(double) * rows * GPIRT_ORD_MAX_WIDTH, st) != hipSuccess ||
        hipMemsetAsync(A.cum, 0, sizeof(double) * rows * (size_t)N, st) != hipSuccess ||
        hipMemsetAsync(A.G, 0, sizeof(double) * ((size_t)Np * (size_t)C * (size_t)m + 2), st) != hipSuccess ||
        hipMemsetAsync(A.window, 0, sizeof(int) * rows, st) != hipSuccess ||
        hipMemsetAsync(A.stat, 0, sizeof(long long) * 4, st) != hipSuccess ||
        hipMemsetAsync(A.hist, 0, sizeof(uint32_t) * rows * Ps, st) != hipSuccess ||
        hipMemsetAsync(A.draws, 0, draw_bytes, st) != hipSuccess) return fail(GPIRT_E_HIP, "the upload");
    if (launch_ord_indicators(st, A.cat, n, m, C, A.Y) != 0 || launch_ord_counts(st, A.cat, n, m, C, A.counts) != 0)
        return fail(GPIRT_E_HIP, "the indicator launch");
    std::vector<double> hb((size_t)(2 * m));
    if (hipMemcpyAsync(hb.data(), s->beta, sizeof(double) * (size_t)(2 * m), hipMemcpyDeviceToHost, st) != hipSuccess ||
        hipStreamSynchronize(st) != hipSuccess) return fail(GPIRT_E_HIP, "reading beta");
    for (int64_t j = 0; j < m; ++j) hb[(size_t)(2 * j)] = 0.0;
    if (hipMemcpyAsync(s->beta, hb.data(), sizeof(double) * (size_t)(2 * m), hipMemcpyHostToDevice, st) != hipSuccess ||
        launch_linear_mean(st, s->theta, n, s->beta, m, s->mu) != 0 ||
        launch_linear_mean(st, s->tstar, N, s->beta, m, s->mu_star) != 0 ||
        hipStreamSynchronize(st) != hipSuccess) return fail(GPIRT_E_HIP, "pinning the intercept");
    A.on = true;
    return 0;
}

int gpirt_sampler_draw_thresholds(gpirt_sampler_t s)
{
    GP_ARG(s && s->initialised);
    OrdState& A = s->ord;
    GP_TRY(needs(A.on, "ordinal responses are", "gpirt_sampler_ordinal_enable"));
    GP_TRY(beta_sync(s));
    s->lp_current = false;
    OrdThrArgs a{};
    a.f = s->f; a.mu = s->mu; a.cat = A.cat; a.counts = A.counts; a.n = s->n; a.m = s->m;
    a.grid = A.d_grid; a.log_prior = A.d_log_prior; a.C = A.C; a.P = A.P; a.W = A.W;
    a.idx = A.idx; a.thr = A.thr; a.lp = A.lp; a.window = A.window; a.stat = A.stat;
    a.seed = s->opt.seed; a.t = A.t + 1; a.item0 = (uint32_t)s->opt.item0;
    hipStream_t st = s->h->stream;
    const bool timed = s->timing;
    if (timed) {
        for (hipEvent_t& t : A.tev) if (!t) GP_HIP(hipEventCreate(&t));
        GP_HIP(hipEventRecord(A.tev[0], st));
    }
    GP_TRY(launch_ord_thresholds(st, a));
    A.t += 1;
    A.lp_W = A.W;
    if (timed) {
        GP_HIP(hipEventRecord(A.tev[1], st));
        GP_HIP(hipEventSynchronize(A.tev[1]));
        float ms = 0.f;
        hipEventElapsedTime(&ms, A.tev[0], A.tev[1]);
        A.last_ms = ms;
    }
    return 0;
}

int gpirt_sampler_ordinal_width(gpirt_sampler_t s, int W)
{
    GP_ARG(s != nullptr);
    GP_TRY(needs(s->ord.on, "ordinal responses are", "gpirt_sampler_ordinal_enable"));
    if (W < 1 || W > GPIRT_ORD_MAX_WIDTH) { set_error("ordinal: window width W = %d, it must lie in 1 .. %d", W, GPIRT_ORD_MAX_WIDTH); return GPIRT_E_ARG; }
    s->ord.W = W;
    return 0;
}

int gpirt_sampler_ordinal_record(gpirt_sampler_t s)
{
// ... 55 lines not shown
    if (!A.on) return 0;
    long long st3[3];
    GP_HIP(hipMemcpyAsync(st3, A.stat, sizeof(st3), hipMemcpyDeviceToHost, s->h->stream));
    GP_HIP(hipStreamSynchronize(s->h->stream));
    out->categories = A.C; out->points = A.P; out->width = A.W; out->lp_width = A.lp_W; out->hi = A.hi; out->last_ms = A.last_ms;
    out->pinned = st3[0]; out->failed = st3[1]; out->updates = st3[2];
    out->planned_draws = A.planned; out->recorded = A.recorded; out->irf_draws = A.irf_draws;
    return 0;
}

int gpirt_sampler_ordinal_fit_enable(gpirt_sampler_t s, int parts)
{
    GP_ARG(s != nullptr);
    const char* me = "gpirt_sampler_ordinal_fit_enable";
    if (!s->initialised) { set_error("%s needs an initialised sampler (gpirt_sampler_init)", me); return GPIRT_E_ARG; }
    OrdState& A = s->ord;
    if (parts == 0)
        return stage_enable(s, &A.fit, ofit_free, false, [] { return 0; });
    GP_TRY(needs(A.on, "ordinal responses are", "gpirt_sampler_ordinal_enable"));
    if (parts < 0 || (parts & ~GPIRT_OFIT_ALL)) {
        set_error("%s: parts = %d has bits outside GPIRT_OFIT_WAIC | GPIRT_OFIT_PRED | GPIRT_OFIT_PPC", me, parts);
        return GPIRT_E_ARG;
    }
    return stage_enable(s, &A.fit, ofit_free, true,
                        [&] { return ofit_alloc(s->h->stream, &A.fit, s->n, s->m, A.C, parts, s->opt.item0, A.cat); });
}

int gpirt_sampler_ordinal_fit_accumulate(gpirt_sampler_t s)
{
    GP_ARG(s && s->initialised);
    OrdState& A = s->ord;
    GP_TRY(needs(A.on && A.fit.on, "the ordinal fit block is", "gpirt_sampler_ordinal_fit_enable"));
    GP_TRY(beta_sync(s));
    return launch_ofit_accumulate(s->h->stream, &A.fit, s->f, s->mu, A.cat, A.thr, s->opt.seed, (uint32_t)s->iter);
}

int gpirt_sampler_ordinal_fit_get(gpirt_sampler_t s, const char* name, void* h_out, int64_t bytes)
{
    GP_ARG(s && name && h_out && bytes >= 0);
    OrdState& A = s->ord;
    GP_TRY(needs(A.on && A.fit.on, "the ordinal fit block is", "gpirt_sampler_ordinal_fit_enable"));
    const int rc = ofit_last_get(s->h->stream, &A.fit, name, h_out, bytes);
    if (rc != 1) return rc;
    GP_TRY(ofit_seal(s->h->stream, &A.fit));
    return ofit_block_get(s->h->stream, A.fit.block, name, h_out, bytes);
}

int gpirt_sampler_ordinal_fit_totals(gpirt_sampler_t s, gpirt_ordinal_fit* out)
{
    GP_ARG(s && out);
    OrdState& A = s->ord;
    GP_TRY(needs(A.on && A.fit.on, "the ordinal fit block is", "gpirt_sampler_ordinal_fit_enable"));
    GP_TRY(ofit_seal(s->h->stream, &A.fit));
    return ofit_block_totals(s->h->stream, A.fit.block, out);
}

int gpirt_sampler_ordinal_fit_state(gpirt_sampler_t s, void** d_block, int64_t* bytes)
{
    GP_ARG(s && d_block && bytes);
    OrdState& A = s->ord;
    GP_TRY(needs(A.on && A.fit.on, "the ordinal fit block is", "gpirt_sampler_ordinal_fit_enable"));
    GP_TRY(ofit_seal(s->h->stream, &A.fit));
    *d_block = A.fit.block;
    *bytes = ofit_state_words(&A.fit) * (int64_t)sizeof(uint64_t);
    return 0;
}

// ... 28 lines not shown
    GP_TRY(aux_join(s));
    s->iter = iter;
    return 0;
}

int gpirt_sampler_check(gpirt_sampler_t s)
{
    GP_ARG(s != nullptr);
    gpirt_handle_t h = s->h;
    hipStream_t st = h->stream;
    GP_TRY(aux_join(s));
    GP_HIP(hipMemcpyAsync(h->h_info, h->d_info, 8 * sizeof(int), hipMemcpyDeviceToHost, st));
    GP_HIP(hipMemcpyAsync(s->h_flags, s->flags, 2 * sizeof(int), hipMemcpyDeviceToHost, st));
    GP_HIP(hipStreamSynchronize(st));
    if (h->h_info[1] != 0) {
        if (!s->factor_fresh || h->cfg.panel == 2) return report_panel_guard(h, h->h_info, st);
        GP_TRY(recover_factor(s));
        GP_HIP(hipMemcpyAsync(h->h_info, h->d_info, 8 * sizeof(int), hipMemcpyDeviceToHost, st));
        GP_HIP(hipStreamSynchronize(st));
        if (h->h_info[1] != 0) return report_panel_guard(h, h->h_info, st);
    }
    if (*h->h_info > 0) {
        set_error("chol(): decomposition failed (leading minor of order %d is not positive definite)", *h->h_info);
        return *h->h_info;
    }
    if (s->h_flags[0] != 0) {
        set_error("sampler state is not finite (flag %d): elliptical slice sampler did not terminate or the R stream window overflowed", s->h_flags[0]);
        return s->h_flags[0];
    }
    if (s->h_flags[1] != 0) return report_degenerate_theta(s, s->h_flags[1]);
    return 0;
}

static int lookup(gpirt_sampler_t s, const char* name, void** p, int64_t* count)
{
    const int64_t n = s->n, m = s->m, N = s->N;
    struct E { const char* k; void* p; int64_t c; } tab[] = {
        { "theta", s->theta, n }, { "f", s->f, n * m }, { "beta", s->beta, 2 * m }, { "mu", s->mu, n * m },
        { "mu_star", s->mu_star, N * m }, { "fstar", s->fstar, N * m }, { "L", s->L, n * n },
        { "logpost", s->logpost, N * n }, { "irf_sum", s->irf_sum, N * m }, { "ess_k", s->ess_k, m },
        { "s", s->s, N }, { "mean", s->mean, N * m }, { "nu", s->NU, n * m }, { "z", s->Z, n * m },
        { "y", s->y, n * m }, { "rs_trace", s->rs_trace, s->rs_trace ? 128 : 0 },
        { "rs_stats", s->rs_ctl, s->rs_ctl ? 8 : 0 },
        { "fstar_full", s->fstar_full, s->fstar_full ? N * s->blk_m : 0 }, { "theta_stage", s->theta_stage, s->theta_stage ? n : 0 },
        { "gbar", s->shape.gbar, s->shape.on ? N * m : 0 },
    };
    for (auto& e : tab)
        if (strcmp(e.k, name) == 0) { *p = e.p; *count = e.c; return 0; }
    set_error("unknown sampler array '%s'", name);
    return GPIRT_E_ARG;
}

int gpirt_sampler_devptr(gpirt_sampler_t s, const char* name, void** d_ptr, int64_t* count)
{
    GP_ARG(s && name && d_ptr && count);
    GP_TRY(lookup(s, name, d_ptr, count));
    if (strcmp(name, "theta") == 0 || strcmp(name, "beta") == 0 || strcmp(name, "mu") == 0) s->mu_linear = false;
    if (strcmp(name, "y") == 0) s->ess_ypk_valid = false;
    if (strcmp(name, "L") == 0) {
        *count = s->ldl * s->n;
        GP_TRY(ensure_dense_factor(s));
    }
    return 0;
}

int gpirt_sampler_ldl(gpirt_sampler_t s, int64_t* ldl)
{
    GP_ARG(s && ldl);
    *ldl = s->ldl;
    return 0;
}

int gpirt_sampler_panel_factor(gpirt_sampler_t s, int64_t p)
{
    GP_ARG(s && s->initialised);
    GP_TRY(ensure_dense_factor(s));
    return potrf_panel_factor(s->h, s->h->stream, s->L, s->n, s->ldl, p, s->ext);
}

int gpirt_sampler_panel_update(gpirt_sampler_t s, int64_t p, int64_t c)
{
    GP_ARG(s && s->initialised);
    GP_TRY(ensure_dense_factor(s));
    return potrf_panel_update(s->h, s->h->stream, s->L, s->n, s->ldl, p, c, s->ext);
}

int gpirt_sampler_panel_copy(gpirt_sampler_t s, int64_t p, double* d_buf, int to_buf)
{
    GP_ARG(s && s->initialised && d_buf);
    GP_TRY(ensure_dense_factor(s));
    return potrf_panel_copy(s->h->stream, s->L, s->n, s->ldl, p, d_buf, to_buf != 0, s->ext);
}

int gpirt_sampler_panel_rows(gpirt_sampler_t s, int64_t* rows)
{
    GP_ARG(s && rows);
    *rows = s->n + s->ext;
    return 0;
}

int gpirt_sampler_ess_pack_draws(gpirt_sampler_t s, int64_t* draws)
{
    GP_ARG(s && draws);
    *draws = s->ess_pack_draws;
    return 0;
}

int gpirt_sampler_nu_lr_draws(gpirt_sampler_t s, int64_t* draws)
{
    GP_ARG(s && draws);
    *draws = s->nu_lr_draws;
    return 0;
}

int gpirt_sampler_fstar_free_draws(gpirt_sampler_t s, int64_t* draws)
{
    GP_ARG(s && draws);
    *draws = s->fstar_free_draws;
    return 0;
}

int gpirt_sampler_factor_lr_count(gpirt_sampler_t s, int64_t* count)
{
    GP_ARG(s && count);
    *count = s->factor_lr_count;
    return 0;
}

int gpirt_sampler_dense_factor_count(gpirt_sampler_t s, int64_t* count)
{
    GP_ARG(s && count);
    *count = s->dense_factor_count;
    return 0;
}

int gpirt_sampler_dense_factor(gpirt_sampler_t s)
{
// ... 76 lines not shown
    GP_ARG(dst && src && dst->initialised && src->initialised && dst->n == src->n && dst->m == src->m && dst->h == src->h);
    if (dst->ord.on || src->ord.on) {
        set_error("gpirt_sampler_copy_state is refused while ordinal responses are on: the categories, thresholds and records are not copied");
        return GPIRT_E_ARG;
    }
    if (dst->ell.on || src->ell.on) {
        set_error("gpirt_sampler_copy_state is not defined while the length-scale update is on (the index and its tables are not copied)");
        return GPIRT_E_ARG;
    }
    if (dst->amp.mode || src->amp.mode) {
        set_error("gpirt_sampler_copy_state is not defined while per-item amplitudes are on (they are not copied)");
        return GPIRT_E_ARG;
    }
    if (dst->pop.mode || src->pop.mode) {
        set_error("gpirt_sampler_copy_state is not defined while a population prior is on (it is not copied)");
        return GPIRT_E_ARG;
    }
    if (dst->kern.family != src->kern.family || dst->kern.length_scale != src->kern.length_scale) {
        set_error("gpirt_sampler_copy_state: the samplers' kernels differ (length_scale %g and %g)", dst->kern.length_scale, src->kern.length_scale);
        return GPIRT_E_ARG;
    }
    hipStream_t st = dst->h->stream;
    const int64_t n = dst->n, m = dst->m, N = dst->N;
    GP_TRY(aux_join(dst)); GP_TRY(aux_join(src));
    GP_TRY(ensure_dense_factor(src));
    dst->L_structured = false;
    dst->lp_current = false;
    dst->mu_linear = false;
    src->factor_fresh = false;
    invalidate_factor_products(dst);
    GP_HIP(hipMemcpyAsync(dst->theta, src->theta, sizeof(double) * (size_t)n, hipMemcpyDeviceToDevice, st));
    GP_HIP(hipMemcpyAsync(dst->f, src->f, sizeof(double) * (size_t)(n * m), hipMemcpyDeviceToDevice, st));
    GP_HIP(hipMemcpyAsync(dst->beta, src->beta, sizeof(double) * (size_t)(2 * m), hipMemcpyDeviceToDevice, st));
    GP_HIP(hipMemcpyAsync(dst->mu, src->mu, sizeof(double) * (size_t)(n * m), hipMemcpyDeviceToDevice, st));
    GP_HIP(hipMemcpyAsync(dst->mu_star, src->mu_star, sizeof(double) * (size_t)(N * m), hipMemcpyDeviceToDevice, st));
    GP_HIP(hipMemcpyAsync(dst->fstar, src->fstar, sizeof(double) * (size_t)(N * m), hipMemcpyDeviceToDevice, st));
    GP_HIP(hipMemcpy2DAsync(dst->L, (size_t)dst->ldl * 8, src->L, (size_t)src->ldl * 8, (size_t)n * 8, (size_t)n,
                            hipMemcpyDeviceToDevice, st));
    dst->rows_valid = false;
    dst->theta_ok = src->theta_ok; dst->theta_alone = src->theta_alone;
    GP_TRY(rebuild_rows(dst));
    dst->iter = src->iter;
    return 0;
}

int gpirt_sampler_get(gpirt_sampler_t s, const char* name, double* h_out, int64_t count)
{
    GP_ARG(s && name && h_out);
    void* p; int64_t c;
    GP_TRY(lookup(s, name, &p, &c));
    GP_ARG(count <= c);
    const size_t esz = strcmp(name, "ess_k") == 0 ? sizeof(int) : sizeof(double);
    GP_TRY(aux_join(s));
    if (strcmp(name, "L") == 0) GP_TRY(ensure_dense_factor(s));
    if (strcmp(name, "L") == 0 && s->ldl != s->n) {
        GP_ARG(count == s->n * s->n);
        GP_HIP(hipMemcpy2DAsync(h_out, (size_t)s->n * 8, p, (size_t)s->ldl * 8, (size_t)s->n * 8, (size_t)s->n,
                                hipMemcpyDeviceToHost, s->h->stream));
    } else {
        GP_HIP(hipMemcpyAsync(h_out, p, esz * (size_t)count, hipMemcpyDeviceToHost, s->h->stream));
    }
    GP_HIP(hipStreamSynchronize(s->h->stream));
    return 0;
}

int gpirt_sampler_set(gpirt_sampler_t s, const char* name, const double* h_in, int64_t count)
{
    GP_ARG(s && name && h_in);
    void* p; int64_t c;
    GP_TRY(lookup(s, name, &p, &c));
    GP_ARG(count <= c && strcmp(name, "ess_k") != 0);
    if (s->ord.on && strcmp(name, "y") == 0)
        GP_TRY(ord_refuse(s, "gpirt_sampler_set(\"y\")", "the categories were checked against y's missing cells at enable"));
    if (s->ord.on && strcmp(name, "beta") == 0)
        for (int64_t q = 0; q < count; q += 2)
            if (h_in[q] != 0.0) GP_TRY(ord_refuse(s, "gpirt_sampler_set(\"beta\") with a non-zero intercept", "the intercept is pinned at 0"));
    GP_TRY(aux_join(s));
    invalidate_factor_products(s);
    s->lp_current = false;
    if (strcmp(name, "theta") == 0 || strcmp(name, "beta") == 0 || strcmp(name, "mu") == 0) s->mu_linear = false;
    if (strcmp(name, "y") == 0) s->ess_ypk_valid = false;
    if (strcmp(name, "L") == 0 || strcmp(name, "theta") == 0) s->rows_valid = false;
    if (strcmp(name, "L") == 0) s->theta_alone = false;
    if (strcmp(name, "L") == 0) {
        if (count < c) GP_TRY(ensure_dense_factor(s));
        s->L_structured = false;
    }
    if (strcmp(name, "theta") == 0) {
        s->theta_alone = true;
        s->theta_ok = count == s->n;
        for (int64_t i = 0; i < count; ++i) s->theta_ok = s->theta_ok && h_in[i] >= -5.0 && h_in[i] <= 5.0;
    }
    if (strcmp(name, "L") == 0 && s->ldl != s->n) {
        GP_ARG(count == s->n * s->n);
        GP_HIP(hipMemcpy2DAsync(p, (size_t)s->ldl * 8, h_in, (size_t)s->n * 8, (size_t)s->n * 8, (size_t)s->n,
                                hipMemcpyHostToDevice, s->h->stream));
    } else {
        GP_HIP(hipMemcpyAsync(p, h_in, sizeof(double) * (size_t)count, hipMemcpyHostToDevice, s->h->stream));
    }
    GP_HIP(hipStreamSynchronize(s->h->stream));
    return 0;
}

int gpirt_sampler_finish_irfs(gpirt_sampler_t s, int sample_iterations, double* h_irfs)
{
    GP_ARG(s && h_irfs);
    const int64_t cnt = s->N * s->m;
    GP_HIP(hipMemcpyAsync(h_irfs, s->irf_sum, sizeof(double) * (size_t)cnt, hipMemcpyDeviceToHost, s->h->stream));
    GP_HIP(hipStreamSynchronize(s->h->stream));
    const double inv = 1.0 / (double)sample_iterations;
    for (int64_t i = 0; i < cnt; ++i) h_irfs[i] = 1.0 / (1.0 + exp(-(h_irfs[i] * inv)));
    return 0;
}

// ... 154 lines not shown
        if (!rc) rc = summary_out();
        g_last_mcmc_fallbacks = h->guard_fallbacks;
        gpirt_sampler_destroy(s);
        drop_handle();
        return rc;
    }

    constexpr int NS = 3;
    auto even = [](size_t c) { return (c + 1) & ~(size_t)1; };
    const size_t off_beta = even((size_t)n), off_f = off_beta + even((size_t)(2 * m)), off_mu = off_f + even((size_t)(n * m));
    const size_t off_gbar = off_mu + even((size_t)(n * m)) + 3 * even((size_t)(N * m));
    const size_t ck_doubles = off_gbar + (s->shape.on ? even((size_t)(N * m)) : 0);
    const size_t off_fstar = off_mu + even((size_t)(n * m)) + even((size_t)(N * m));
    double* ck[NS] = { nullptr, nullptr, nullptr };
    hipEvent_t ev_flags[NS] = {}, ev_copied[NS] = {};
    bool copy_pending[NS] = { false, false, false };
    int copy_slot[NS] = { 0, 0, 0 };
    std::vector<double> th_stage[NS];
    hipStream_t copy_stream = nullptr;
    int* h_poll = nullptr;
    auto fail_hip = [&](const char* what) { set_error("%s failed in gpirt_mcmc", what); return (int)GPIRT_E_HIP; };
    if (!rc) {
        bool ok = hipStreamCreateWithFlags(&copy_stream, hipStreamNonBlocking) == hipSuccess &&
                  hipHostMalloc(&h_poll, NS * 16 * sizeof(int), hipHostMallocDefault) == hipSuccess;
        for (int q = 0; q < NS && ok; ++q) {
            ok = hipMalloc(&ck[q], ck_doubles * sizeof(double)) == hipSuccess &&
                 hipEventCreateWithFlags(&ev_flags[q], hipEventDisableTiming) == hipSuccess &&
                 hipEventCreateWithFlags(&ev_copied[q], hipEventDisableTiming) == hipSuccess;
            th_stage[q].resize((size_t)n);
        }
        if (!ok) rc = fail_hip("allocation");
    }
    struct Part { double* p; size_t cnt; };
    auto parts = [&]() {
        std::vector<Part> v{ { s->theta, (size_t)n }, { s->beta, (size_t)(2 * m) }, { s->f, (size_t)(n * m) },
                             { s->mu, (size_t)(n * m) }, { s->mu_star, (size_t)(N * m) }, { s->fstar, (size_t)(N * m) },
                             { s->irf_sum, (size_t)(N * m) } };
        if (s->shape.on) v.push_back(Part{ s->shape.gbar, (size_t)(N * m) });
        return v;
    };
    auto save_ckpt = [&](int k) -> int {
        const int q = k % NS;
        hipStream_t st = h->stream;
        if (beta_sync(s) != 0) return fail_hip("draw_beta join");
        if (copy_pending[q] && hipStreamWaitEvent(st, ev_copied[q], 0) != hipSuccess) return fail_hip("hipStreamWaitEvent");
        double* d = ck[q];
        for (const Part& pt : parts()) {
            if (hipMemcpyAsync(d, pt.p, pt.cnt * sizeof(double), hipMemcpyDeviceToDevice, st) != hipSuccess) return fail_hip("checkpoint");
            d += even(pt.cnt);
        }
        if (hipMemcpyAsync(h_poll + 16 * q, h->d_info, 8 * sizeof(int), hipMemcpyDeviceToHost, st) != hipSuccess ||
            hipMemcpyAsync(h_poll + 16 * q + 8, s->flags, 2 * sizeof(int), hipMemcpyDeviceToHost, st) != hipSuccess ||
            hipEventRecord(ev_flags[q], st) != hipSuccess)
            return fail_hip("flag read-back");
        return 0;
    };
    auto finish_store = [&](int q) -> int {
        if (!copy_pending[q]) return 0;
        if (hipEventSynchronize(ev_copied[q]) != hipSuccess) return fail_hip("draw copy");
        const int slot = copy_slot[q];
        if (h_theta_draws)
            for (int64_t i = 0; i < n; ++i) h_theta_draws[slot + i * (int64_t)(S_it + 1)] = th_stage[q][(size_t)i];
        copy_pending[q] = false;
        return 0;
    };
    auto start_store = [&](int k) -> int {
        const int q = k % NS, slot = k - B_it;
        GP_TRY(finish_store(q));
        const double* d = ck[q];
        GP_TRY(accumulate_run(s, DrawView{ d, d + off_beta, d + off_f, d + off_mu, d + off_fstar, d + off_gbar, (uint32_t)k }));
        if (!h_theta_draws && !h_beta_draws && !h_f_draws) return 0;
        if ((h_theta_draws && hipMemcpyAsync(th_stage[q].data(), d, sizeof(double) * (size_t)n, hipMemcpyDeviceToHost, copy_stream) != hipSuccess) ||
            (h_beta_draws && hipMemcpyAsync(h_beta_draws + (int64_t)slot * 2 * m, d + off_beta, sizeof(double) * (size_t)(2 * m), hipMemcpyDeviceToHost, copy_stream) != hipSuccess) ||
            (h_f_draws && hipMemcpyAsync(h_f_draws + (int64_t)slot * n * m, d + off_f, sizeof(double) * (size_t)(n * m), hipMemcpyDeviceToHost, copy_stream) != hipSuccess) ||
            hipEventRecord(ev_copied[q], copy_stream) != hipSuccess)
            return fail_hip("draw copy");
        copy_pending[q] = true; copy_slot[q] = slot;
        return 0;
    };
    auto rollback = [&](int k) -> int {
        hipStream_t st = h->stream;
        if (hipStreamSynchronize(st) != hipSuccess) return fail_hip("hipStreamSynchronize");
        if (h->side) hipStreamSynchronize(h->side);
        if (s->haux) hipStreamSynchronize(s->haux->stream);
        s->beta_deferred = false; s->beta_pending = false; s->prep_pending = false; s->z_filled_iter = 0;
        const double* d = ck[k % NS];
        for (const Part& pt : parts()) {
            if (hipMemcpyAsync(pt.p, d, pt.cnt * sizeof(double), hipMemcpyDeviceToDevice, st) != hipSuccess) return fail_hip("rollback");
            d += even(pt.cnt);
        }
        if (hipMemsetAsync(s->flags, 0, 4 * sizeof(int), st) != hipSuccess) return fail_hip("rollback");
        s->mu_linear = false;
        s->iter = k;
        return recover_factor(s);
    };
    s->sticky_info = true;
    const int panel_mode = h->cfg.panel;
    int it = 0, verified = 0, fallback_until = 0, last_fallback = -1;
    if (!rc) rc = save_ckpt(0);
    if (!rc && hipEventSynchronize(ev_flags[0]) != hipSuccess) rc = fail_hip("hipEventSynchronize");
    while (!rc && verified < total) {
        if (it < total && verified >= it - 1) {
            if (ticked(it, total)) { set_error("interrupted"); rc = GPIRT_E_INTERRUPT; break; }
            h->cfg.panel = (it < fallback_until) ? 2 : panel_mode;
            if (h->aux) h->aux->cfg.panel = h->cfg.panel;
            rc = gpirt_sampler_step(s);
            h->cfg.panel = panel_mode;
            if (h->aux) h->aux->cfg.panel = panel_mode;
            if (!rc && it >= B_it) rc = gpirt_sampler_accumulate_irf(s);
            if (!rc) rc = save_ckpt(it + 1);
            ++it;
            continue;
        }
        const int k = verified + 1, q = k % NS;
        if (hipEventSynchronize(ev_flags[q]) != hipSuccess) { rc = fail_hip("hipEventSynchronize"); break; }
        const int* w = h_poll + 16 * q;
        if (w[1] != 0) {
            if (panel_mode == 2 || last_fallback == verified) { rc = report_panel_guard(h, w, h->stream); break; }
            rc = rollback(verified);
            last_fallback = verified; fallback_until = it; it = verified;
// ... 316 lines not shown
```

gpirt_amd/csrc/stages.hip:

```cpp
#include "common.h"
#include "kernels.h"
#include "ll_fast.h"

namespace gpirt {

namespace {

#define GP_LN_SQRT_2PI 0.918938533204672741780329736406

__device__ __forceinline__ double r_rnorm(double mu, double sd, double z, bool& consumes)
{
    consumes = false;
    if (mu != mu || !isfinite(sd) || sd < 0.0) return __builtin_nan("");
    if (sd == 0.0 || !isfinite(mu)) return mu;
    consumes = true;
    return mu + sd * z;
}

__device__ __forceinline__ double r_dnorm_log(double x, double mu, double sd)
{
    const double z = fabs((x - mu) / sd);
    return -(GP_LN_SQRT_2PI + 0.5 * z * z + log(sd));
}

// ... 282 lines not shown
}

#define DB_COEF(v) double b0 = (v)[0], b1 = (v)[1]; uint32_t lv = live, ng = neg; asm volatile("" : "+v"(b0), "+v"(b1), "+v"(lv), "+v"(ng))
#define DB_KEEP(e) (0ull - (uint64_t)((lv >> (e)) & 1u))
#define DB_ARG(e) __longlong_as_double(__double_as_longlong(F[e] + (b0 + T[e] * b1)) ^ (long long)((uint64_t)((ng >> (e)) & 1u) << 63))
#define DB_TERM(e, fn) __longlong_as_double(__double_as_longlong(fn(DB_ARG(e))) & (long long)DB_KEEP(e))
#define DB_SCREEN_PASS(v)                                                    \
    {                                                                        \
        DB_COEF(v);                                                          \
        acc = 0.0;                                                           \
        tmax = 0.0;                                                          \
        _Pragma("unroll") for (int e = 0; e < EPT; ++e) {                    \
            const double term = DB_TERM(e, ll_term_screen);                  \
            acc += term;                                                     \
            tmax = fmax(tmax, term);                                         \
            if ((e & 3) == 3) __builtin_amdgcn_sched_barrier(0);             \
        }                                                                    \
    }
#define DB_FULL_PASS(v)                                                      \
    {                                                                        \
        DB_COEF(v);                                                          \
        acc = 0.0;                                                           \
        _Pragma("unroll") for (int e = 0; e < EPT; ++e) {                    \
            acc += DB_TERM(e, ll_term);                                      \
            __builtin_amdgcn_sched_barrier(0);                               \
        }                                                                    \
    }
__device__ __forceinline__ double db_uniform(double v)
{
    const int lo = __builtin_amdgcn_readfirstlane(__double2loint(v)), hi = __builtin_amdgcn_readfirstlane(__double2hiint(v));
    return __hiloint2double(hi, lo);
}

template <int EPT>
__global__ __launch_bounds__(256) void draw_beta_reg_kernel(BetaArgs a)
{
    static_assert(EPT <= 32, "one bit per row in the masks");
    __shared__ double red[4];
    const int64_t j = blockIdx.x;
    const int n = (int)a.n;
    const int t = threadIdx.x;
    const double* __restrict__ fj = a.f + j * a.n;
    const double* __restrict__ yj = a.y + j * a.n;
    const double* __restrict__ th = a.theta;
    const uint32_t item = a.item0 + (uint32_t)j;
    double F[EPT], T[EPT];
    uint32_t live = 0, neg = 0;
#pragma unroll
    for (int e = 0; e < EPT; ++e) {
        const int i = t + 256 * e;
        const int ic = i < n ? i : n - 1;
        const double yy = yj[ic];
        F[e] = fj[ic];
        T[e] = th[ic];
        live |= (uint32_t)(i < n && yy == yy) << e;
        neg |= (uint32_t)(yy < 0.0) << e;
        if ((e & 7) == 7) __builtin_amdgcn_sched_barrier(0);
    }
    double cv[2] = { a.beta[0 + 2 * j], a.beta[1 + 2 * j] };
    double pv[2] = { cv[0], cv[1] };
    const double band = LL_SCREEN_ERR * (double)n;
    double kept_ll = 0.0;
    bool have_kept = false;
    double kept_s = 0.0;
    int kept_ovf = 0;
    double acc, tmax;
    for (int k = 0; k < 2; ++k) {
        const double step = a.step[k + 2 * j];
        const double z = qnorm_as241(item_uniform(a.seed, a.iter, GPIRT_ST_BETA, item, (uint32_t)(2 * k)));
        bool consumes;
        pv[k] = db_uniform(r_rnorm(cv[k], step, z, consumes));
        const double pm = a.pm[k + 2 * j], ps = a.ps[k + 2 * j];
        const double pv_prior = db_uniform(r_dnorm_log(pv[k], pm, ps));
        const double cv_prior = db_uniform(r_dnorm_log(cv[k], pm, ps));
        DB_SCREEN_PASS(pv);
        const double s_p = db_uniform(block_sum_256(acc, red));
        const int ovf_p = __syncthreads_or(tmax > 709.0);
        double s_c = kept_s;
        int ovf_c = kept_ovf;
        if (k == 0) {
            DB_SCREEN_PASS(cv);
            s_c = db_uniform(block_sum_256(acc, red));
            ovf_c = __syncthreads_or(tmax > 709.0);
        }
        const double u = item_uniform(a.seed, a.iter, GPIRT_ST_BETA, item, (uint32_t)(2 * k + 1));
        const double log_u = db_uniform(log(u));
        const double r_s = (pv_prior - cv_prior) - s_p + s_c;
        int verdict = 0;
        if (r_s - 2.0 * band > log_u) verdict = 1;
        else if (r_s + 2.0 * band < log_u) verdict = -1;
        if (ovf_p | ovf_c) verdict = 0;
        const bool full = verdict == 0;
        double pv_ll = 0.0, cv_ll = 0.0;
        if (full) {
            DB_FULL_PASS(pv);
            pv_ll = db_uniform(-block_sum_256(acc, red));
            if (k == 1 && have_kept) {
                cv_ll = kept_ll;
            } else {
                DB_FULL_PASS(cv);
                cv_ll = db_uniform(-block_sum_256(acc, red));
            }
            const double r = pv_prior + pv_ll - cv_prior - cv_ll;
            verdict = (log_u < r) ? 1 : -1;
        }
        if (a.path && t == 0) a.path[k + 2 * j] = full ? 1 : 0;
        if (verdict > 0) { cv[k] = pv[k]; kept_ll = pv_ll; kept_s = s_p; kept_ovf = ovf_p; }
        else { pv[k] = cv[k]; kept_ll = cv_ll; kept_s = s_c; kept_ovf = ovf_c; }
        have_kept = full;
    }
    if (t == 0) { a.beta[0 + 2 * j] = cv[0]; a.beta[1 + 2 * j] = cv[1]; }
    if (a.mu) {
        double* __restrict__ mj = a.mu + j * a.n;
        int t2 = t;
        asm volatile("" : "+v"(t2));
#pragma unroll
        for (int e = 0; e < EPT; ++e) {
            const int i = t2 + 256 * e;
            if (i < n) mj[i] = cv[0] + T[e] * cv[1];
            if ((e & 7) == 7) __builtin_amdgcn_sched_barrier(0);
        }
    }
    if (a.mu_star)
        for (int64_t i = t; i < a.N; i += 256)
            a.mu_star[i + j * a.N] = cv[0] + (-5.0 + (double)i * 0.01) * cv[1];
}
#undef DB_COEF
#undef DB_KEEP
#undef DB_ARG
#undef DB_TERM
#undef DB_SCREEN_PASS
#undef DB_FULL_PASS

__global__ void linear_mean_kernel(const double* __restrict__ x, int64_t n, const double* __restrict__ beta,
                                   int64_t m, double* __restrict__ mu)
{
    const int64_t total = n * m;
    for (int64_t g = (int64_t)blockIdx.x * blockDim.x + threadIdx.x; g < total;
         g += (int64_t)gridDim.x * blockDim.x) {
        const int64_t j = g / n, i = g - j * n;
        mu[g] = beta[0 + 2 * j] + x[i] * beta[1 + 2 * j];
    }
}

__global__ void axpy_kernel(double* __restrict__ acc, const double* __restrict__ x, int64_t count)
{
    for (int64_t g = (int64_t)blockIdx.x * blockDim.x + threadIdx.x; g < count;
         g += (int64_t)gridDim.x * blockDim.x)
        acc[g] += x[g];
}

inline unsigned grid_for(int64_t total)
{
    int64_t b = (total + 255) / 256;
    if (b > 8192) b = 8192;
    if (b < 1) b = 1;
    return (unsigned)b;
}

}

int launch_colnorm_s(hipStream_t stream, const double* tmp, int64_t n, int64_t N, int64_t ld, double* s)
{
    if (N <= 0) return 0;
    hipLaunchKernelGGL(colnorm_s_kernel, dim3((unsigned)N), dim3(256), 0, stream, tmp, n, ld, s);
    GP_HIP(hipGetLastError());
// ... 33 lines not shown

int launch_loglik_terms(hipStream_t stream, const double* fstar, int64_t N, int64_t m, double* Gpm, int64_t ldg, const int* run_if)
{
    const unsigned blocks = run_if ? (grid_for(N * m) < 256u ? grid_for(N * m) : 256u) : grid_for(N * m);
    hipLaunchKernelGGL(loglik_terms_kernel, dim3(blocks), dim3(256), 0, stream, fstar, N, m, Gpm, ldg, run_if);
    GP_HIP(hipGetLastError());
    return 0;
}

int launch_theta_nan_fix(hipStream_t stream, const double* Gpm, int64_t ldg, const double* Ypm, int64_t n, int64_t m,
                         double* lp, int64_t N, int64_t ldlp, const int* run_if)
{
    if (N * n <= 0) return 0;
    const unsigned blocks = run_if ? (grid_for(N * n) < 256u ? grid_for(N * n) : 256u) : grid_for(N * n);
    hipLaunchKernelGGL(theta_nan_fix_kernel, dim3(blocks), dim3(256), 0, stream, Gpm, ldg, Ypm, n, m, lp, N, ldlp, run_if);
    GP_HIP(hipGetLastError());
    return 0;
}

int launch_theta_sample(hipStream_t stream, const ThetaArgs& a)
{
    if (a.n <= 0) return 0;
    if (a.N > 1024) { set_error("theta grid larger than 1024 points is not supported"); return GPIRT_E_ARG; }
    if (a.log_prior && a.codes) hipLaunchKernelGGL(theta_sample_kernel<true>, dim3((unsigned)a.n), dim3(256), 0, stream, a);
    else hipLaunchKernelGGL(theta_sample_kernel<false>, dim3((unsigned)a.n), dim3(256), 0, stream, a);
    GP_HIP(hipGetLastError());
    return 0;
}

int launch_draw_beta(hipStream_t stream, const BetaArgs& a)
{
    if (a.m <= 0) return 0;
    const bool reg = a.screen == 1 && a.U == nullptr && a.n >= 1 && a.n <= 256 * 32;
    if (reg && a.n <= 256 * 8) hipLaunchKernelGGL(draw_beta_reg_kernel<8>, dim3((unsigned)a.m), dim3(256), 0, stream, a);
    else if (reg && a.n <= 256 * 16) hipLaunchKernelGGL(draw_beta_reg_kernel<16>, dim3((unsigned)a.m), dim3(256), 0, stream, a);
    else if (reg) hipLaunchKernelGGL(draw_beta_reg_kernel<32>, dim3((unsigned)a.m), dim3(256), 0, stream, a);
    else hipLaunchKernelGGL(draw_beta_kernel, dim3((unsigned)a.m), dim3(256), 0, stream, a);
    GP_HIP(hipGetLastError());
    return 0;
}

int launch_linear_mean(hipStream_t stream, const double* x, int64_t n, const double* beta, int64_t m, double* mu)
{
    if (n * m <= 0) return 0;
    hipLaunchKernelGGL(linear_mean_kernel, dim3(grid_for(n * m)), dim3(256), 0, stream, x, n, beta, m, mu);
    GP_HIP(hipGetLastError());
    return 0;
}

__global__ __launch_bounds__(256) void transpose_kernel(const double* __restrict__ in, int64_t rows, int64_t cols, int64_t ldi,
                                                        double* __restrict__ out, int64_t ldo)
{
    __shared__ double tile[32][33];
    const int tx = threadIdx.x & 31, ty = threadIdx.x >> 5;
    const int64_t r0 = (int64_t)blockIdx.x * 32, c0 = (int64_t)blockIdx.y * 32;
#pragma unroll
    for (int k = 0; k < 4; ++k) {
        const int64_t r = r0 + tx, c = c0 + ty + 8 * k;
        tile[ty + 8 * k][tx] = (r < rows && c < cols) ? in[r + c * ldi] : 0.0;
    }
    __syncthreads();
#pragma unroll
    for (int k = 0; k < 4; ++k) {
        const int64_t c = c0 + tx, r = r0 + ty + 8 * k;
        if (r < rows && c < cols) out[c + r * ldo] = tile[tx][ty + 8 * k];
    }
}

int launch_transpose(hipStream_t stream, const double* in, int64_t rows, int64_t cols, int64_t ldi, double* out, int64_t ldo)
{
// ... 17 lines not shown
```

gpirt_amd/ops.py:

```python
from __future__ import annotations

import ctypes as C

import numpy as np
import torch

from . import _lib
from ._lib import NGRID, check


def colmajor(n: int, m: int, device="cuda", fill=None) -> torch.Tensor:
    base = torch.empty((m, n), dtype=torch.float64, device=device)
    if fill is not None:
        base.fill_(fill)
    return base.T


def to_device(a, device="cuda") -> torch.Tensor:
    a = np.asarray(a, dtype=np.float64)
    if a.ndim == 1:
        return torch.from_numpy(np.ascontiguousarray(a)).to(device)
    if a.ndim != 2:
        raise ValueError("expected a vector or a matrix")
    return torch.from_numpy(np.ascontiguousarray(a.T)).to(device).T
# ... 233 lines not shown
        n, m = f.shape
        out = colmajor(NGRID, m, f.device)
        s = torch.empty(NGRID, dtype=torch.float64, device=f.device)
        mean = colmajor(NGRID, m, f.device)
        check(self.lib.gpirt_draw_fstar(self._h, _p(f), _p(theta), _p(L), _ld(L), _p(mu_star), n, m, seed, it,
                                        int(fused), _p(out), _p(s), _p(mean)))
        return out, s, mean

    def draw_theta(self, y, fstar, seed: int, it: int, stabilise: bool = True):
        n, m = y.shape
        out = torch.empty(n, dtype=torch.float64, device=y.device)
        deg = torch.zeros(1, dtype=torch.int32, device=y.device)
        check(self.lib.gpirt_draw_theta(self._h, _p(y), _p(fstar), n, m, seed, it, int(stabilise), _p(out), _p(deg)))
        return out, int(deg.item())

    def theta_logpost(self, y, fstar):
        n, m = y.shape
        out = colmajor(NGRID, n, y.device)
        fb = C.c_int(0)
        check(self.lib.gpirt_debug_theta_logpost(self._h, _p(y), _p(fstar), n, m, _p(out), C.byref(fb)))
        return out, fb.value

    def draw_beta(self, beta, theta, y, f, pm, ps, step, seed: int, it: int, paths: bool = False):
        n, m = y.shape
        if not paths:
            check(self.lib.gpirt_draw_beta(self._h, _p(beta), _p(theta), _p(y), _p(f), _p(pm), _p(ps), _p(step),
                                           n, m, seed, it))
            return beta
        path = torch.full((m, 2), -1, dtype=torch.int32, device=y.device)
        check(self.lib.gpirt_draw_beta_paths(self._h, _p(beta), _p(theta), _p(y), _p(f), _p(pm), _p(ps), _p(step),
                                             n, m, seed, it, _p(path)))
        return beta, path.t()

    def prof_enable(self, on: bool):
        check(self.lib.gpirt_prof_enable(self._h, int(on)))

    def prof_trailing(self, reset: bool = False):
        ms = C.c_double()
        n = C.c_int64()
        fl = C.c_double()
        check(self.lib.gpirt_prof_trailing(self._h, int(reset), C.byref(ms), C.byref(n), C.byref(fl)))
        return ms.value, n.value, fl.value

    SYRK_CLASSES = ("trailing_128tile", "trailing_64tile", "in_panel_update")

    def prof_syrk(self, reset: bool = False) -> dict:
        out = {}
        for cls, name in enumerate(self.SYRK_CLASSES):
            ms, n, fl, by = C.c_double(), C.c_int64(), C.c_double(), C.c_double()
            check(self.lib.gpirt_prof_syrk_bytes(self._h, cls, C.byref(by)))
            check(self.lib.gpirt_prof_syrk(self._h, cls, int(reset), C.byref(ms), C.byref(n), C.byref(fl)))
            out[name] = (ms.value, n.value, fl.value, by.value)
        return out

    OTHER_CLASSES = {3: "draw_f_trmm", 4: "replay_products", 5: "theta_int8_product"}

    def prof_other(self, reset: bool = False) -> dict:
        out = {}
        for cls, name in self.OTHER_CLASSES.items():
            ms, n, fl, by = C.c_double(), C.c_int64(), C.c_double(), C.c_double()
            check(self.lib.gpirt_prof_syrk_bytes(self._h, cls, C.byref(by)))
            check(self.lib.gpirt_prof_syrk(self._h, cls, int(reset), C.byref(ms), C.byref(n), C.byref(fl)))
            out[name] = (ms.value, n.value, fl.value, by.value)
        return out


# ... 41 lines not shown
```

gpirt_amd/sampler.py:

```python
from __future__ import annotations

import ctypes as C

import numpy as np

from . import _lib
from ._lib import NGRID, RNG_ITEM, RNG_RSTREAM, Options, check
from .response_matrix import as_response_matrix

_dp = C.POINTER(C.c_double)


def _f64(a):
    return np.asfortranarray(np.array(a, dtype=np.float64))


def _ptr(a):
    return a.ctypes.data_as(_dp)


def _options(rng, seed, theta_stabilise, fstar_fused, device, item0=0, m_total=0, kernel_fp32=False,
             kstar_rank=0, factor_structured=False) -> Options:
    o = _lib.default_options()
    o.rng_kind = RNG_RSTREAM if rng == "reference" else RNG_ITEM
# ... 521 lines not shown

    def panel_update(self, p: int, c: int):
        check(self.lib.gpirt_sampler_panel_update(self._s, int(p), int(c)))

    def panel_copy(self, p: int, buf, to_buf: bool):
        check(self.lib.gpirt_sampler_panel_copy(self._s, int(p), C.c_void_p(buf.data_ptr()), int(bool(to_buf))))

    @property
    def subpanel_width(self) -> int:
        return int(self.lib.gpirt_potrf_subpanel_width(int(self.n)))

    def panel_factor_part(self, p: int, half: int):
        check(self.lib.gpirt_sampler_panel_factor_part(self._s, int(p), int(half)))

    def panel_update_part(self, p: int, c: int, part: int):
        check(self.lib.gpirt_sampler_panel_update_part(self._s, int(p), int(c), int(part)))

    def panel_copy_part(self, p: int, half: int, buf, to_buf: bool):
        check(self.lib.gpirt_sampler_panel_copy_part(self._s, int(p), int(half), C.c_void_p(buf.data_ptr()), buf.numel(),
                                                     int(bool(to_buf))))

    def streams_busy(self) -> int:
        b = C.c_int()
        check(self.lib.gpirt_debug_streams_busy(self.handle.ptr, C.byref(b)))
        return b.value

    @property
    def nu_lr_draws(self) -> int:
        r = C.c_int64()
        check(self.lib.gpirt_sampler_nu_lr_draws(self._s, C.byref(r)))
        return r.value

    @property
    def ess_pack_draws(self) -> int:
        r = C.c_int64()
        check(self.lib.gpirt_sampler_ess_pack_draws(self._s, C.byref(r)))
        return r.value

    @property
    def fstar_free_draws(self) -> int:
        r = C.c_int64()
        check(self.lib.gpirt_sampler_fstar_free_draws(self._s, C.byref(r)))
        return r.value

    @property
    def factor_lr_count(self) -> int:
        r = C.c_int64()
        check(self.lib.gpirt_sampler_factor_lr_count(self._s, C.byref(r)))
        return int(r.value)

    @property
    def dense_factor_count(self) -> int:
        r = C.c_int64()
        check(self.lib.gpirt_sampler_dense_factor_count(self._s, C.byref(r)))
        return int(r.value)

    def dense_factor(self):
        self._call("gpirt_sampler_dense_factor")

    def factor_lr_parts(self) -> list:
        out = np.empty((self.n, 512), dtype=np.float64)
        check(self.lib.gpirt_sampler_factor_lr_parts(self._s, C.c_void_p(out.ctypes.data), out.size))
        return [out[p:p + 512, :min(512, self.n - p)].T.copy() for p in range(0, self.n, 512)]

    @property
    def factor_lr_width(self) -> int:
# ... 1083 lines not shown
```

include/gpirt_hip.h:

```cpp
#ifndef GPIRT_HIP_H
#define GPIRT_HIP_H

#include <stddef.h>
#include <stdint.h>

#ifdef __cplusplus
extern "C" {
#endif

#define GPIRT_NGRID 1001
#define GPIRT_JITTER 0.001

enum {
    GPIRT_OK          = 0,
    GPIRT_E_ARG       = -1,
    GPIRT_E_HIP       = -2,
    GPIRT_E_NODEVICE  = -3,
    GPIRT_E_ALLOC     = -4,
    GPIRT_E_RNG       = -5,
    GPIRT_E_INTERRUPT = -6,
    GPIRT_E_NUMERIC   = -7
};

enum { GPIRT_RNG_RSTREAM = 0, GPIRT_RNG_ITEM = 1 };
// ... 68 lines not shown
int gpirt_potrf_panel_factor_part(gpirt_handle_t h, double* d_A, int64_t n, int64_t lda, int64_t p, int half);
int gpirt_potrf_panel_update_part(gpirt_handle_t h, double* d_A, int64_t n, int64_t lda, int64_t p, int64_t c, int part);
int gpirt_potrf_panel_copy_part(gpirt_handle_t h, double* d_A, int64_t n, int64_t lda, int64_t p, int half, double* d_buf,
                                int64_t buf_doubles, int to_buf);
int gpirt_debug_streams_busy(gpirt_handle_t h, int* busy);
int gpirt_debug_panel_trace(gpirt_handle_t h, int64_t k0, long long* host_out, int64_t count);
int gpirt_debug_ll_term(gpirt_handle_t h, const double* d_a, int64_t n, double* d_out, int fast);
int gpirt_debug_theta_logpost(gpirt_handle_t h, const double* d_y, const double* d_fstar, int64_t n, int64_t m,
                              double* d_logpost_out, int* fell_back);
int gpirt_debug_theta_clock(gpirt_handle_t h, const double* d_y, const double* d_fstar, int64_t n, int64_t m,
                            long long* host_stamps, int64_t count);

int gpirt_trmm_lz(gpirt_handle_t h, const double* d_L, int64_t n, int64_t ldl, const double* d_Z,
                  int64_t m, int64_t ldz, double* d_out, int64_t ldo);

int gpirt_trsm_lower(gpirt_handle_t h, const double* d_L, int64_t n, int64_t ldl, double* d_B,
                     int64_t nrhs, int64_t ldb, int trans);

int gpirt_gemm(gpirt_handle_t h, int ta, int tb, int64_t M, int64_t N, int64_t K, double alpha,
               const double* d_A, int64_t lda, const double* d_B, int64_t ldb, double beta,
               double* d_C, int64_t ldc);

int gpirt_ll_bar(gpirt_handle_t h, const double* d_f, const double* d_y, const double* d_mu,
                 int64_t n, int64_t m, double* d_out);

int gpirt_draw_f(gpirt_handle_t h, double* d_f, const double* d_y, const double* d_L, int64_t ldl,
                 const double* d_mu, int64_t n, int64_t m, uint64_t seed, uint32_t iter,
                 int* d_k_out);

int gpirt_draw_f_linear(gpirt_handle_t h, double* d_f, const double* d_y, const double* d_L, int64_t ldl,
                        const double* d_theta, const double* d_beta, int64_t n, int64_t m, uint64_t seed,
                        uint32_t iter, int* d_k_out);
int gpirt_sampler_ess_pack_draws(gpirt_sampler_t s, int64_t* draws);

int gpirt_draw_fstar(gpirt_handle_t h, const double* d_f, const double* d_theta, const double* d_L,
                     int64_t ldl, const double* d_mu_star, int64_t n, int64_t m, uint64_t seed,
                     uint32_t iter, int fused, double* d_out, double* d_s_out, double* d_mean_out);

int gpirt_draw_theta(gpirt_handle_t h, const double* d_y, const double* d_fstar, int64_t n,
                     int64_t m, uint64_t seed, uint32_t iter, int stabilise, double* d_theta_out,
                     int* d_degenerate);

int gpirt_draw_beta(gpirt_handle_t h, double* d_beta, const double* d_theta, const double* d_y,
                    const double* d_f, const double* d_prior_means, const double* d_prior_sds,
                    const double* d_step_sizes, int64_t n, int64_t m, uint64_t seed, uint32_t iter);
int gpirt_draw_beta_paths(gpirt_handle_t h, double* d_beta, const double* d_theta, const double* d_y,
                          const double* d_f, const double* d_prior_means, const double* d_prior_sds,
                          const double* d_step_sizes, int64_t n, int64_t m, uint64_t seed, uint32_t iter, int* d_path);

int gpirt_item_uniforms(gpirt_handle_t h, uint64_t seed, uint32_t iter, uint32_t stage,
                        uint32_t item0, int64_t n_items, int64_t n_index, double* d_out);
int gpirt_item_normals(gpirt_handle_t h, uint64_t seed, uint32_t iter, uint32_t stage,
                       uint32_t item0, int64_t n_items, int64_t n_index, double* d_out);

typedef struct gpirt_rstream_s* gpirt_rstream_t;
int gpirt_rstream_create(gpirt_rstream_t* r, uint32_t seed);
int gpirt_rstream_from_state(gpirt_rstream_t* r, const uint32_t mt[624], int mti);
int gpirt_rstream_get_state(gpirt_rstream_t r, uint32_t mt[624], int* mti);
int gpirt_rstream_destroy(gpirt_rstream_t r);
int gpirt_rstream_unif(gpirt_rstream_t r, double* h_out, int64_t n);
int gpirt_rstream_norm(gpirt_rstream_t r, double* h_out, int64_t n);

typedef int (*gpirt_tick_fn)(void* ctx, int iter, int total);

typedef struct gpirt_options {
    int      rng_kind;
// ... 1045 lines not shown
```

Baseline: 1204.

## Read packed y bitmasks in beta register kernel and optionally defer forming mu

Adds a kernel that packs each item's responses into per-thread live/negative bitmasks once, cached on the sampler. The beta register kernel can then read these instead of streaming the full double-precision y matrix on every draw, which cuts memory traffic. A second mode, selected by GPIRT_BETA_PACK=1 and off by default, skips writing the n×m mu matrix. It instead stores theta and the beta pairs and rebuilds mu lazily through a settle hook when a consumer (ESS, ellipse, summaries, checkpoints) asks for it. This adds bookkeeping state and must keep mu consistent across every consumer.

Measured after the change: 1218, median of 3. No clear change (+1.2%).

```diff
diff --git a/gpirt_amd/_lib.py b/gpirt_amd/_lib.py
--- a/gpirt_amd/_lib.py
+++ b/gpirt_amd/_lib.py
@@ -726,6 +726,9 @@
     "gpirt_sampler_ldl": (_i32, [_vp, C.POINTER(_i64)]),
     "gpirt_sampler_nu_lr_draws": (_i32, [_vp, C.POINTER(_i64)]),
     "gpirt_sampler_ess_pack_draws": (_i32, [_vp, C.POINTER(_i64)]),
+    "gpirt_sampler_beta_pack_draws": (_i32, [_vp, C.POINTER(_i64)]),
+    "gpirt_beta_pack": (_i32, [_vp, _vp, _i64, _i64, _vp]),
+    "gpirt_draw_beta_packed": (_i32, [_vp, _vp, _vp, _vp, _vp, _vp, _vp, _vp, _i64, _i64, _u64, _u32, _vp, _vp, _vp, _vp]),
     "gpirt_sampler_nu_lr_rows": (_i32, [_vp, _vp, _i64]),
     "gpirt_sampler_fstar_free_draws": (_i32, [_vp, C.POINTER(_i64)]),
     "gpirt_sampler_factor_lr_count": (_i32, [_vp, C.POINTER(_i64)]),
diff --git a/gpirt_amd/csrc/api.hip b/gpirt_amd/csrc/api.hip
--- a/gpirt_amd/csrc/api.hip
+++ b/gpirt_amd/csrc/api.hip
@@ -44,6 +44,7 @@
         d.beta_screen = env_value("GPIRT_BETA_SCREEN", d.beta_screen);
         d.zfill_compact = env_value("GPIRT_ZFILL_COMPACT", d.zfill_compact);
         d.ess_pack = env_value("GPIRT_ESS_PACK", d.ess_pack);
+        d.beta_pack = env_value("GPIRT_BETA_PACK", d.beta_pack);
         if (d.nbo < 64) d.nbo = 1024;
         if (d.nbp != 0 && d.nbp < 64) d.nbp = 512;
         return d;
@@ -165,7 +166,7 @@
 
 extern "C" {
 
-int gpirt_version(void) { return 143; }
+int gpirt_version(void) { return 144; }
 
 const char* gpirt_last_error(void) { return g_err; }
 
@@ -295,6 +296,7 @@
         { "GPIRT_BETA_SCREEN", &h->cfg.beta_screen, false },
         { "GPIRT_ZFILL_COMPACT", &h->cfg.zfill_compact, false },
         { "GPIRT_ESS_PACK", &h->cfg.ess_pack, false },
+        { "GPIRT_BETA_PACK", &h->cfg.beta_pack, false },
     };
     for (auto& e : tab)
         if (strcmp(e.k, name) == 0) { if (read_only) *read_only = e.ro; return e.p; }
@@ -836,6 +838,37 @@
     return draw_beta_op(h, d_beta, d_theta, d_y, d_f, d_pm, d_ps, d_step, n, m, seed, iter, d_path);
 }
 
+int gpirt_beta_pack(gpirt_handle_t h, const double* d_y, int64_t n, int64_t m, uint32_t* d_ypk)
+{
+    GP_ARG(h && d_y && d_ypk && m >= 0);
+    if (n < 1 || n > 8192) { set_error("gpirt_beta_pack: n = %lld, the register kernel takes 1 <= n <= 8192", (long long)n); return GPIRT_E_ARG; }
+    return launch_beta_pack(h->stream, d_y, n, m, d_ypk);
+}
+
+int gpirt_draw_beta_packed(gpirt_handle_t h, double* d_beta, const double* d_theta, const double* d_y,
+                           const double* d_f, const double* d_pm, const double* d_ps, const double* d_step,
+                           int64_t n, int64_t m, uint64_t seed, uint32_t iter, uint32_t* d_ypk, double* d_mu,
+                           double* d_beta_mu, int* d_path)
+{
+    GP_ARG(h && d_beta && d_theta && d_y && d_f && d_pm && d_ps && d_step && d_ypk && m >= 0);
+    if (n < 1 || n > 8192) { set_error("gpirt_draw_beta_packed: n = %lld, the register kernel takes 1 <= n <= 8192", (long long)n); return GPIRT_E_ARG; }
+    if (m == 0) return 0;
+    GP_TRY(ensure_work(h, 8 * sizeof(double)));
+    int* bad = reinterpret_cast<int*>(h->d_work);
+    GP_HIP(hipMemsetAsync(bad, 0, sizeof(int), h->stream));
+    GP_TRY(launch_check_y(h->stream, d_y, n * m, bad));
+    GP_HIP(hipMemcpyAsync(h->h_info, bad, sizeof(int), hipMemcpyDeviceToHost, h->stream));
+    GP_HIP(hipStreamSynchronize(h->stream));
+    if (*h->h_info != 0) { set_error("gpirt_draw_beta_packed: y must be +1, -1 or NaN"); return GPIRT_E_ARG; }
+    GP_TRY(launch_beta_pack(h->stream, d_y, n, m, d_ypk));
+    BetaArgs a{};
+    a.beta = d_beta; a.theta = d_theta; a.y = d_y; a.f = d_f; a.pm = d_pm; a.ps = d_ps; a.step = d_step;
+    a.n = n; a.m = m; a.N = GPIRT_NGRID; a.mu = d_mu; a.mu_star = nullptr;
+    a.seed = seed; a.iter = iter; a.item0 = 0; a.U = nullptr; a.path = d_path;
+    a.screen = 1; a.ypk = d_ypk; a.beta_mu = d_beta_mu;
+    return launch_draw_beta(h->stream, a);
+}
+
 int gpirt_prof_enable(gpirt_handle_t h, int on)
 {
     GP_ARG(h != nullptr);
diff --git a/gpirt_amd/csrc/common.h b/gpirt_amd/csrc/common.h
--- a/gpirt_amd/csrc/common.h
+++ b/gpirt_amd/csrc/common.h
@@ -70,6 +70,7 @@
     int  flr_narrow = 1;
     int  beta_screen = 1;
     int  ess_pack = 1;
+    int  beta_pack = 3;
     int  zfill_compact = 1;
     int  rs_predict = 1;
     int  guard_verbose = 0;
diff --git a/gpirt_amd/csrc/kernels.h b/gpirt_amd/csrc/kernels.h
--- a/gpirt_amd/csrc/kernels.h
+++ b/gpirt_amd/csrc/kernels.h
@@ -436,8 +436,10 @@
     const double* U; uint64_t* pos; const uint64_t* item_off; uint64_t cap; int* err;
     int screen;
     int* path;
+    const uint32_t* ypk; double* beta_mu; double* theta_mu;
 };
 int launch_draw_beta(hipStream_t stream, const BetaArgs& a);
+int launch_beta_pack(hipStream_t stream, const double* y, int64_t n, int64_t m, uint32_t* out);
 int launch_linear_mean(hipStream_t stream, const double* x, int64_t n, const double* beta, int64_t m, double* mu);
 
 int prof_pair_begin(gpirt_handle_t h, hipStream_t stream, ProfPair& pp);
diff --git a/gpirt_amd/csrc/sampler.hip b/gpirt_amd/csrc/sampler.hip
--- a/gpirt_amd/csrc/sampler.hip
+++ b/gpirt_amd/csrc/sampler.hip
@@ -144,7 +144,7 @@
     KernelSpec kern;
     RStream* rs = nullptr;
     double *y = nullptr, *Ypm = nullptr, *theta = nullptr, *theta_new = nullptr, *f = nullptr,
-           *Z = nullptr, *NU = nullptr, *beta = nullptr, *mu = nullptr, *mu_star = nullptr,
+           *Z = nullptr, *NU = nullptr, *beta = nullptr, *mu_buf = nullptr, *mu_star = nullptr,
            *fstar = nullptr, *L = nullptr, *tstar = nullptr, *kstar = nullptr, *rhs = nullptr,
            *mean = nullptr, *s = nullptr, *Gpm = nullptr, *logpost = nullptr, *irf_sum = nullptr,
            *pm = nullptr, *ps = nullptr, *step = nullptr;
@@ -242,6 +242,11 @@
     uint32_t* ess_ypk = nullptr;
     bool ess_ypk_valid = false;
     int64_t ess_pack_draws = 0;
+    double *theta_mu = nullptr, *beta_mu = nullptr;
+    bool mu_unstored = false, mu_wanted = false;
+    uint32_t* beta_ypk = nullptr;
+    bool beta_ypk_valid = false;
+    int64_t beta_pack_draws = 0;
 };
 
 namespace {
@@ -268,6 +273,25 @@
 }
 
 inline bool stream_mode(const gpirt_sampler_s* s) { return s->opt.rng_kind == GPIRT_RNG_RSTREAM; }
+
+int mu_settle(gpirt_sampler_s* s, hipStream_t stream)
+{
+    if (!s->mu_unstored) return 0;
+    GP_TRY(launch_linear_mean(stream, s->theta_mu, s->n, s->beta_mu, s->m, s->mu_buf));
+    s->mu_unstored = false;
+    return 0;
+}
+double* mu_ptr(gpirt_sampler_s* s, hipStream_t stream)
+{
+    s->mu_wanted = true;
+    return mu_settle(s, stream) == 0 ? s->mu_buf : nullptr;
+}
+double* mu_whole(gpirt_sampler_s* s)
+{
+    s->mu_unstored = false;
+    return s->mu_buf;
+}
+#define GP_MU(var, s, stream) double* var = mu_ptr((s), (stream)); if (!var) return GPIRT_E_HIP
 
 int report_degenerate_theta(gpirt_sampler_s* s, int count);
 
@@ -557,14 +581,15 @@
         if (prep && !early && !free) GP_HIP(hipEventRecord(s->ev_trmm, st));
         if (s->ord.on) {
             EssOrdArgs a{};
-            a.f = s->f; a.nu = s->NU; a.mu = s->mu; a.cat = s->ord.cat; a.thr = s->ord.thr; a.counts = s->ord.counts;
+            GP_MU(mu, s, st);
+            a.f = s->f; a.nu = s->NU; a.mu = mu; a.cat = s->ord.cat; a.thr = s->ord.thr; a.counts = s->ord.counts;
             a.C = s->ord.C; a.n = n; a.m = m; a.k_out = s->ess_k; a.err = s->flags;
             a.seed = s->opt.seed; a.iter = iter; a.item0 = (uint32_t)s->opt.item0;
             a.screen = h->cfg.ess_screen == 1;
             GP_TRY(launch_ess_ord(st, a));
         } else {
         EssArgs a{};
-        a.f = s->f; a.nu = s->NU; a.y = s->y; a.mu = s->mu; a.n = n; a.m = m; a.k_out = s->ess_k;
+        a.f = s->f; a.nu = s->NU; a.y = s->y; a.n = n; a.m = m; a.k_out = s->ess_k;
         a.err = s->flags; a.seed = s->opt.seed; a.iter = iter; a.item0 = (uint32_t)s->opt.item0;
         a.ll_exact = h->cfg.ll_exact;
         a.screen = h->cfg.ess_screen == 1;
@@ -573,6 +598,9 @@
             a.ypk = s->ess_ypk; a.theta = s->theta; a.beta = s->beta;
             a.grid = h->cfg.ess_pack == 3 ? 2 * h->n_cu : 0;
             s->ess_pack_draws += 1;
+        } else {
+            GP_MU(mu, s, st);
+            a.mu = mu;
         }
         GP_TRY(launch_ess(st, a));
         }
@@ -592,11 +620,12 @@
         }
         return 0;
     }
+    GP_MU(mu, s, st);
     auto plain_item = [&](int64_t j) -> int {
         GP_TRY(launch_rstream_normals(st, s->U, s->pos, 0, n, 1, s->Z));
         GP_TRY(launch_trmv_lower(st, s->L, n, s->ldl, s->Z, s->NU + n, s->NU));
         EssArgs a{};
-        a.f = s->f + j * n; a.nu = s->NU; a.y = s->y + j * n; a.mu = s->mu + j * n; a.n = n; a.m = 1;
+        a.f = s->f + j * n; a.nu = s->NU; a.y = s->y + j * n; a.mu = mu + j * n; a.n = n; a.m = 1;
         a.k_out = s->ess_k + j; a.err = s->flags; a.item0 = (uint32_t)j;
         a.U = s->U; a.pos = s->pos; a.cap = s->U_cap;
         return launch_ess(st, a);
@@ -616,7 +645,7 @@
         if (h->rs_cand_limit < a.lim1) a.lim1 = h->rs_cand_limit;
         if (h->rs_cand_limit < a.lim2) a.lim2 = h->rs_cand_limit;
     }
-    a.f = s->f; a.y = s->y; a.mu = s->mu; a.partial = s->rs_partial; a.flags = s->rs_flags;
+    a.f = s->f; a.y = s->y; a.mu = mu; a.partial = s->rs_partial; a.flags = s->rs_flags;
     GP_TRY(launch_rs3_begin(st, a, (uint64_t)m * (2ull * (uint64_t)n + 2ull) + 512ull * (uint64_t)m + 4096ull));
     int64_t pass = 0, done = 0;
     int64_t one_phase = 0;
@@ -669,7 +698,7 @@
             GP_TRY(launch_rs_gather(st, s->Nrm, s->posv, s->anchorP, n, done, m, s->Z));
             GP_TRY(launch_gemm(h, st, false, false, TRI_A_LOWER, n, mc, n, 1.0, s->L, s->ldl, s->Z, n, 0.0, s->NU, n));
             RsVerifyArgs v{};
-            v.f = s->f; v.nu = s->NU; v.y = s->y; v.mu = s->mu; v.n = n; v.m = m; v.j0 = done;
+            v.f = s->f; v.nu = s->NU; v.y = s->y; v.mu = mu; v.n = n; v.m = m; v.j0 = done;
             v.U = s->U; v.cap = s->U_cap; v.posv = s->posv; v.anchorP = s->anchorP;
             v.kv = s->rs_kv; v.used = s->rs_used; v.ierr = s->rs_ierr;
             GP_TRY(launch_rs_verify(st, v));
@@ -900,20 +929,37 @@
 {
     s->lp_current = false;
     s->mu_linear = !s->ord.on;
+    const bool wanted = s->mu_wanted;
+    s->mu_wanted = false;
     if (s->ord.on) {
         BetaOrdArgs a{};
         a.beta = s->beta; a.theta = s->theta; a.cat = s->ord.cat; a.f = s->f; a.thr = s->ord.thr; a.pm = s->pm; a.ps = s->ps;
-        a.step = s->step; a.C = s->ord.C; a.n = s->n; a.m = s->m; a.N = s->N; a.mu = s->mu; a.mu_star = s->mu_star;
+        a.step = s->step; a.C = s->ord.C; a.n = s->n; a.m = s->m; a.N = s->N; a.mu = mu_whole(s); a.mu_star = s->mu_star;
         a.seed = s->opt.seed; a.iter = (uint32_t)(s->iter + 1); a.item0 = (uint32_t)s->opt.item0;
         return launch_draw_beta_ord(st, a);
     }
     BetaArgs a{};
     a.beta = s->beta; a.theta = s->theta; a.y = s->y; a.f = s->f; a.pm = s->pm; a.ps = s->ps;
-    a.step = s->step; a.n = s->n; a.m = s->m; a.N = s->N; a.mu = s->mu; a.mu_star = s->mu_star;
+    a.step = s->step; a.n = s->n; a.m = s->m; a.N = s->N; a.mu_star = s->mu_star;
     a.seed = s->opt.seed; a.iter = (uint32_t)(s->iter + 1); a.item0 = (uint32_t)s->opt.item0;
     a.err = s->flags;
     a.screen = s->h->cfg.beta_screen == 1;
     if (stream_mode(s)) { a.U = s->U; a.pos = s->pos; a.item_off = s->beta_off; a.cap = s->U_cap; }
+    const int bp = s->h->cfg.beta_pack;
+    const bool packed = bp != 2 && a.screen == 1 && !stream_mode(s) && s->beta_ypk && s->n >= 1 && s->n <= 8192;
+    const bool lazy = packed && bp == 1 && !wanted && s->theta_mu && s->ess_ypk && !s->opt.kernel_fp32
+                      && ess_pack_eligible(s->n) && s->h->cfg.ess_pack != 2;
+    if (packed) {
+        if (!s->beta_ypk_valid) { GP_TRY(launch_beta_pack(st, s->y, s->n, s->m, s->beta_ypk)); s->beta_ypk_valid = true; }
+        a.ypk = s->beta_ypk;
+    }
+    if (lazy) {
+        a.beta_mu = s->beta_mu; a.theta_mu = s->theta_mu;
+        s->mu_unstored = true;
+        s->beta_pack_draws += 1;
+    } else {
+        a.mu = mu_whole(s);
+    }
     GP_TRY(launch_draw_beta(st, a));
     if (stream_mode(s)) GP_TRY(launch_advance_pos(st, s->pos, s->beta_total));
     return 0;
@@ -1305,11 +1351,13 @@
     c.factorisations += 1;
     tick(3);
     const double lp_diff = e.log_prior[(size_t)kp] - e.log_prior[(size_t)e.k], log_u = log(u1);
+    double* mu = mu_ptr(s, st);
+    if (!mu && !rc) rc = GPIRT_E_HIP;
     for (int attempt = 0; !rc; ++attempt) {
         if (kind == ELL_WHITENED) {
             rc = launch_gemm(h, st, false, false, TRI_A_LOWER, n, m, n, 1.0, s->L, s->ldl, s->NU, n, 0.0, e.fprop, n);
             tick(4);
-            if (!rc) rc = launch_ell_delta(st, s->f, e.fprop, s->mu, s->y, n, m, e.delta, e.nonfin);
+            if (!rc) rc = launch_ell_delta(st, s->f, e.fprop, mu, s->y, n, m, e.delta, e.nonfin);
             tick(5);
             if (!rc) rc = launch_ell_decide(st, e.delta, e.nonfin, m, lp_diff, log_u, h->d_info, e.rec, e.flag);
             tick(6);
@@ -1536,18 +1584,24 @@
 }
 
 struct DrawView { const double *theta, *beta, *f, *mu, *fstar, *gbar; uint32_t iter; };
-DrawView live_view(gpirt_sampler_t s) { return { s->theta, s->beta, s->f, s->mu, s->fstar, s->shape.gbar, (uint32_t)s->iter }; }
-
-int acc_summary(gpirt_sampler_t s, const DrawView& v) { return launch_summary_accumulate(s->h->stream, &s->sum, v.theta, v.beta, v.f, v.mu, s->y, v.fstar); }
-int acc_ppc(gpirt_sampler_t s, const DrawView& v) { return launch_ppc_accumulate(s->h->stream, &s->ppc, v.f, v.mu, s->y, s->opt.seed, v.iter, v.theta); }
+DrawView live_view(gpirt_sampler_t s) { return { s->theta, s->beta, s->f, nullptr, s->fstar, s->shape.gbar, (uint32_t)s->iter }; }
+const double* view_mu(gpirt_sampler_t s, const DrawView& v)
+{
+    if (v.mu) return v.mu;
+    if (beta_sync(s) != 0) return nullptr;
+    return mu_ptr(s, s->h->stream);
+}
+
+int acc_summary(gpirt_sampler_t s, const DrawView& v) { const double* mu = view_mu(s, v); if (!mu) return GPIRT_E_HIP; return launch_summary_accumulate(s->h->stream, &s->sum, v.theta, v.beta, v.f, mu, s->y, v.fstar); }
+int acc_ppc(gpirt_sampler_t s, const DrawView& v) { const double* mu = view_mu(s, v); if (!mu) return GPIRT_E_HIP; return launch_ppc_accumulate(s->h->stream, &s->ppc, v.f, mu, s->y, s->opt.seed, v.iter, v.theta); }
 int acc_rank(gpirt_sampler_t s, const DrawView& v) { return launch_rank_accumulate(s->h->stream, &s->rank, v.theta); }
 int acc_score(gpirt_sampler_t s, const DrawView& v) { return launch_score_accumulate(s->h, s->h->stream, &s->score, v.fstar); }
 int acc_shape(gpirt_sampler_t s, const DrawView& v) { return launch_shape_accumulate(s->h->stream, &s->shape, v.gbar); }
 int acc_sumscore(gpirt_sampler_t s, const DrawView& v) { return launch_sumscore_accumulate(s->h->stream, &s->sumscore, v.fstar); }
 int acc_equate(gpirt_sampler_t s, const DrawView& v) { return launch_equate_accumulate(s->h, s->h->stream, &s->equate, v.fstar); }
-int acc_loo(gpirt_sampler_t s, const DrawView& v) { return launch_loo_accumulate(s->h->stream, &s->loo, v.f, v.mu); }
-int acc_acf(gpirt_sampler_t s, const DrawView& v) { return launch_acf_accumulate(s->h->stream, &s->acf, v.theta, v.beta, v.f, v.mu, s->y); }
-int acc_groups(gpirt_sampler_t s, const DrawView& v) { return launch_groups_accumulate(s->h->stream, &s->groups, v.theta, v.f, v.mu, s->y); }
+int acc_loo(gpirt_sampler_t s, const DrawView& v) { const double* mu = view_mu(s, v); if (!mu) return GPIRT_E_HIP; return launch_loo_accumulate(s->h->stream, &s->loo, v.f, mu); }
+int acc_acf(gpirt_sampler_t s, const DrawView& v) { const double* mu = view_mu(s, v); if (!mu) return GPIRT_E_HIP; return launch_acf_accumulate(s->h->stream, &s->acf, v.theta, v.beta, v.f, mu, s->y); }
+int acc_groups(gpirt_sampler_t s, const DrawView& v) { const double* mu = view_mu(s, v); if (!mu) return GPIRT_E_HIP; return launch_groups_accumulate(s->h->stream, &s->groups, v.theta, v.f, mu, s->y); }
 
 int accumulate_run(gpirt_sampler_t s, const DrawView& v)
 {
@@ -1664,7 +1718,7 @@
     s->theta_ok = true;
     for (int64_t i = 0; i < n; ++i) s->theta_ok = s->theta_ok && h_theta0[i] >= -5.0 && h_theta0[i] <= 5.0;
     s->nu_kern_ok = nu_kernel_ok(s->kern);
-    GP_A(s->mu, n * m);      GP_A(s->mu_star, N * m + 1); GP_A(s->fstar, N * m + 1); GP_A(s->L, s->ldl * n);
+    GP_A(s->mu_buf, n * m);      GP_A(s->mu_star, N * m + 1); GP_A(s->fstar, N * m + 1); GP_A(s->L, s->ldl * n);
     GP_A(s->tstar, N + 1);   GP_A(s->rhs, n * (N + m) + 2); GP_A(s->mean, N * m + 1); GP_A(s->s, N + 1);
     GP_A(s->Gpm, ((N + 127) / 128 * 128) * 2 * m + 2); GP_A(s->logpost, N * n + 2); GP_A(s->irf_sum, N * m + 1);
     if (hipMemsetAsync(s->Gpm, 0, sizeof(double) * (size_t)(((N + 127) / 128 * 128) * 2 * m + 2), st) != hipSuccess) {
@@ -1676,6 +1730,11 @@
         rc = dalloc(s, &s->ess_ypk, (size_t)(512 * m), false);
         if (rc) { gpirt_sampler_destroy(s); return rc; }
     }
+    if (!stream_mode(s) && n >= 1 && n <= 8192) {
+        rc = dalloc(s, &s->beta_ypk, (size_t)(512 * m), false);
+        if (rc) { gpirt_sampler_destroy(s); return rc; }
+    }
+    if (s->ess_ypk) { GP_A(s->theta_mu, n); GP_A(s->beta_mu, 2 * m); }
     if (!s->opt.fstar_fused) GP_A(s->kstar, n * N + 2);
     if (s->node_off >= 0) {
         GP_A(s->nu_nodes, NU_LR_RANK); GP_A(s->nu_wts, NU_LR_RANK);
@@ -1822,6 +1881,7 @@
     launch_indicators(st, s->y, n, m, s->Ypm);
     launch_tf_indicators(st, s->y, n, n, m, s->tfd, s->tf_y8);
     if (s->ess_ypk) { launch_ess_pack(st, s->y, n, m, s->ess_ypk); s->ess_ypk_valid = true; }
+    if (s->beta_ypk && h->cfg.beta_pack != 2) { launch_beta_pack(st, s->y, n, m, s->beta_ypk); s->beta_ypk_valid = true; }
     if (hipStreamSynchronize(st) != hipSuccess || hipGetLastError() != hipSuccess) {
         set_error("sampler upload failed"); gpirt_sampler_destroy(s); return GPIRT_E_HIP;
     }
@@ -1970,7 +2030,7 @@
         GP_HIP(hipMemcpyAsync(s->beta, b.data(), sizeof(double) * b.size(), hipMemcpyHostToDevice, st));
         GP_HIP(hipStreamSynchronize(st));
     }
-    GP_TRY(launch_linear_mean(st, s->theta, n, s->beta, m, s->mu));
+    GP_TRY(launch_linear_mean(st, s->theta, n, s->beta, m, mu_whole(s)));
     s->mu_linear = true;
     GP_TRY(launch_linear_mean(st, s->tstar, N, s->beta, m, s->mu_star));
     GP_TRY(do_draw_fstar(s, 0));
@@ -3104,7 +3164,8 @@
     GP_TRY(needs(A.mode == 2, "the amplitude update is", "gpirt_sampler_amp_enable"));
     GP_TRY(beta_sync(s));
     AmpUpdateArgs a{};
-    a.f = s->f; a.mu = s->mu; a.y = s->y; a.n = s->n; a.m = s->m;
+    GP_MU(mu, s, s->h->stream);
+    a.f = s->f; a.mu = mu; a.y = s->y; a.n = s->n; a.m = s->m;
     a.grid = A.d_grid; a.log_prior = A.d_log_prior; a.P = A.P;
     a.idx = A.idx; a.width = A.width; a.amp = A.amp; a.counts = A.counts; a.rec = A.rec;
     a.seed = s->opt.seed; a.t = A.t + 1; a.item0 = (uint32_t)s->opt.item0;
@@ -3350,7 +3411,8 @@
     GP_TRY(smooth_factor(s));
     AmpCentredArgs a = A.ca;
     a.F = s->sf.F; a.live = s->sf.live; a.r = s->sf.r;
-    a.f = s->f; a.mu = s->mu; a.y = s->y; a.n = s->n; a.m = s->m;
+    GP_MU(mu, s, s->h->stream);
+    a.f = s->f; a.mu = mu; a.y = s->y; a.n = s->n; a.m = s->m;
     a.theta = s->theta; a.eps = GPIRT_JITTER;
     a.H = s->NU;
     a.grid = A.d_grid; a.log_prior = A.d_log_prior; a.P = A.P;
@@ -3477,7 +3539,8 @@
     GP_TRY(beta_centred_alloc(s));
     GP_TRY(smooth_factor(s));
     BetaCentredArgs a = Bc.a;
-    a.f = s->f; a.beta = s->beta; a.mu = s->mu; a.mu_star = s->mu_star; a.n = s->n; a.m = s->m; a.N = s->N;
+    GP_MU(mu, s, s->h->stream);
+    a.f = s->f; a.beta = s->beta; a.mu = mu; a.mu_star = s->mu_star; a.n = s->n; a.m = s->m; a.N = s->N;
     a.theta = s->theta; a.tstar = s->tstar; a.pm = s->pm; a.ps = s->ps;
     a.amp = s->amp.mode ? s->amp.amp : nullptr;
     a.F = s->sf.F; a.eps = GPIRT_JITTER;
@@ -3652,7 +3715,8 @@
     }
     ScaleState& Sc = s->sc;
     ScaleArgs a = Sc.a;
-    a.beta = s->beta; a.mu = s->mu; a.mu_star = s->mu_star; a.fstar = s->fstar; a.logpost = s->logpost;
+    GP_MU(mu, s, s->h->stream);
+    a.beta = s->beta; a.mu = mu; a.mu_star = s->mu_star; a.fstar = s->fstar; a.logpost = s->logpost;
     a.gbar = s->shape.on ? s->shape.gbar : nullptr;
     a.n = s->n; a.m = s->m; a.N = s->N; a.theta = s->theta; a.pm = s->pm; a.ps = s->ps;
     if (s->pop.mode) { a.log_prior = s->pop.log_prior; a.codes = s->pop.codes; }
@@ -4125,7 +4189,7 @@
         hipStreamSynchronize(st) != hipSuccess) return fail(GPIRT_E_HIP, "reading beta");
     for (int64_t j = 0; j < m; ++j) hb[(size_t)(2 * j)] = 0.0;
     if (hipMemcpyAsync(s->beta, hb.data(), sizeof(double) * (size_t)(2 * m), hipMemcpyHostToDevice, st) != hipSuccess ||
-        launch_linear_mean(st, s->theta, n, s->beta, m, s->mu) != 0 ||
+        launch_linear_mean(st, s->theta, n, s->beta, m, mu_whole(s)) != 0 ||
         launch_linear_mean(st, s->tstar, N, s->beta, m, s->mu_star) != 0 ||
         hipStreamSynchronize(st) != hipSuccess) return fail(GPIRT_E_HIP, "pinning the intercept");
     A.on = true;
@@ -4140,7 +4204,8 @@
     GP_TRY(beta_sync(s));
     s->lp_current = false;
     OrdThrArgs a{};
-    a.f = s->f; a.mu = s->mu; a.cat = A.cat; a.counts = A.counts; a.n = s->n; a.m = s->m;
+    GP_MU(mu, s, s->h->stream);
+    a.f = s->f; a.mu = mu; a.cat = A.cat; a.counts = A.counts; a.n = s->n; a.m = s->m;
     a.grid = A.d_grid; a.log_prior = A.d_log_prior; a.C = A.C; a.P = A.P; a.W = A.W;
     a.idx = A.idx; a.thr = A.thr; a.lp = A.lp; a.window = A.window; a.stat = A.stat;
     a.seed = s->opt.seed; a.t = A.t + 1; a.item0 = (uint32_t)s->opt.item0;
@@ -4262,7 +4327,8 @@
     OrdState& A = s->ord;
     GP_TRY(needs(A.on && A.fit.on, "the ordinal fit block is", "gpirt_sampler_ordinal_fit_enable"));
     GP_TRY(beta_sync(s));
-    return launch_ofit_accumulate(s->h->stream, &A.fit, s->f, s->mu, A.cat, A.thr, s->opt.seed, (uint32_t)s->iter);
+    GP_MU(mu, s, s->h->stream);
+    return launch_ofit_accumulate(s->h->stream, &A.fit, s->f, mu, A.cat, A.thr, s->opt.seed, (uint32_t)s->iter);
 }
 
 int gpirt_sampler_ordinal_fit_get(gpirt_sampler_t s, const char* name, void* h_out, int64_t bytes)
@@ -4357,11 +4423,17 @@
     return 0;
 }
 
+static int lookup_mu(gpirt_sampler_t s, const char* name)
+{
+    if (strcmp(name, "mu") != 0) return 0;
+    return mu_ptr(s, s->h->stream) ? 0 : GPIRT_E_HIP;
+}
+
 static int lookup(gpirt_sampler_t s, const char* name, void** p, int64_t* count)
 {
     const int64_t n = s->n, m = s->m, N = s->N;
     struct E { const char* k; void* p; int64_t c; } tab[] = {
-        { "theta", s->theta, n }, { "f", s->f, n * m }, { "beta", s->beta, 2 * m }, { "mu", s->mu, n * m },
+        { "theta", s->theta, n }, { "f", s->f, n * m }, { "beta", s->beta, 2 * m }, { "mu", s->mu_buf, n * m },
         { "mu_star", s->mu_star, N * m }, { "fstar", s->fstar, N * m }, { "L", s->L, n * n },
         { "logpost", s->logpost, N * n }, { "irf_sum", s->irf_sum, N * m }, { "ess_k", s->ess_k, m },
         { "s", s->s, N }, { "mean", s->mean, N * m }, { "nu", s->NU, n * m }, { "z", s->Z, n * m },
@@ -4380,8 +4452,13 @@
 {
     GP_ARG(s && name && d_ptr && count);
     GP_TRY(lookup(s, name, d_ptr, count));
+    if (strcmp(name, "mu") == 0 && s->beta_pending) {
+        GP_HIP(hipStreamWaitEvent(s->h->stream, s->ev_beta, 0));
+        s->beta_pending = false;
+    }
+    GP_TRY(lookup_mu(s, name));
     if (strcmp(name, "theta") == 0 || strcmp(name, "beta") == 0 || strcmp(name, "mu") == 0) s->mu_linear = false;
-    if (strcmp(name, "y") == 0) s->ess_ypk_valid = false;
+    if (strcmp(name, "y") == 0) s->ess_ypk_valid = s->beta_ypk_valid = false;
     if (strcmp(name, "L") == 0) {
         *count = s->ldl * s->n;
         GP_TRY(ensure_dense_factor(s));
@@ -4428,6 +4505,13 @@
 {
     GP_ARG(s && draws);
     *draws = s->ess_pack_draws;
+    return 0;
+}
+
+int gpirt_sampler_beta_pack_draws(gpirt_sampler_t s, int64_t* draws)
+{
+    GP_ARG(s && draws);
+    *draws = s->beta_pack_draws;
     return 0;
 }
 
@@ -4570,7 +4654,11 @@
     GP_HIP(hipMemcpyAsync(dst->theta, src->theta, sizeof(double) * (size_t)n, hipMemcpyDeviceToDevice, st));
     GP_HIP(hipMemcpyAsync(dst->f, src->f, sizeof(double) * (size_t)(n * m), hipMemcpyDeviceToDevice, st));
     GP_HIP(hipMemcpyAsync(dst->beta, src->beta, sizeof(double) * (size_t)(2 * m), hipMemcpyDeviceToDevice, st));
-    GP_HIP(hipMemcpyAsync(dst->mu, src->mu, sizeof(double) * (size_t)(n * m), hipMemcpyDeviceToDevice, st));
+    {
+        const double* src_mu = mu_ptr(src, st);
+        if (!src_mu) return GPIRT_E_HIP;
+        GP_HIP(hipMemcpyAsync(mu_whole(dst), src_mu, sizeof(double) * (size_t)(n * m), hipMemcpyDeviceToDevice, st));
+    }
     GP_HIP(hipMemcpyAsync(dst->mu_star, src->mu_star, sizeof(double) * (size_t)(N * m), hipMemcpyDeviceToDevice, st));
     GP_HIP(hipMemcpyAsync(dst->fstar, src->fstar, sizeof(double) * (size_t)(N * m), hipMemcpyDeviceToDevice, st));
     GP_HIP(hipMemcpy2DAsync(dst->L, (size_t)dst->ldl * 8, src->L, (size_t)src->ldl * 8, (size_t)n * 8, (size_t)n,
@@ -4590,6 +4678,7 @@
     GP_ARG(count <= c);
     const size_t esz = strcmp(name, "ess_k") == 0 ? sizeof(int) : sizeof(double);
     GP_TRY(aux_join(s));
+    GP_TRY(lookup_mu(s, name));
     if (strcmp(name, "L") == 0) GP_TRY(ensure_dense_factor(s));
     if (strcmp(name, "L") == 0 && s->ldl != s->n) {
         GP_ARG(count == s->n * s->n);
@@ -4614,10 +4703,11 @@
         for (int64_t q = 0; q < count; q += 2)
             if (h_in[q] != 0.0) GP_TRY(ord_refuse(s, "gpirt_sampler_set(\"beta\") with a non-zero intercept", "the intercept is pinned at 0"));
     GP_TRY(aux_join(s));
+    GP_TRY(lookup_mu(s, name));
     invalidate_factor_products(s);
     s->lp_current = false;
     if (strcmp(name, "theta") == 0 || strcmp(name, "beta") == 0 || strcmp(name, "mu") == 0) s->mu_linear = false;
-    if (strcmp(name, "y") == 0) s->ess_ypk_valid = false;
+    if (strcmp(name, "y") == 0) s->ess_ypk_valid = s->beta_ypk_valid = false;
     if (strcmp(name, "L") == 0 || strcmp(name, "theta") == 0) s->rows_valid = false;
     if (strcmp(name, "L") == 0) s->theta_alone = false;
     if (strcmp(name, "L") == 0) {
@@ -4838,9 +4928,9 @@
         if (!ok) rc = fail_hip("allocation");
     }
     struct Part { double* p; size_t cnt; };
-    auto parts = [&]() {
+    auto parts = [&](bool restore) {
         std::vector<Part> v{ { s->theta, (size_t)n }, { s->beta, (size_t)(2 * m) }, { s->f, (size_t)(n * m) },
-                             { s->mu, (size_t)(n * m) }, { s->mu_star, (size_t)(N * m) }, { s->fstar, (size_t)(N * m) },
+                             { restore ? mu_whole(s) : mu_ptr(s, h->stream), (size_t)(n * m) }, { s->mu_star, (size_t)(N * m) }, { s->fstar, (size_t)(N * m) },
                              { s->irf_sum, (size_t)(N * m) } };
         if (s->shape.on) v.push_back(Part{ s->shape.gbar, (size_t)(N * m) });
         return v;
@@ -4851,7 +4941,8 @@
         if (beta_sync(s) != 0) return fail_hip("draw_beta join");
         if (copy_pending[q] && hipStreamWaitEvent(st, ev_copied[q], 0) != hipSuccess) return fail_hip("hipStreamWaitEvent");
         double* d = ck[q];
-        for (const Part& pt : parts()) {
+        for (const Part& pt : parts(false)) {
+            if (!pt.p) return fail_hip("forming mu");
             if (hipMemcpyAsync(d, pt.p, pt.cnt * sizeof(double), hipMemcpyDeviceToDevice, st) != hipSuccess) return fail_hip("checkpoint");
             d += even(pt.cnt);
         }
@@ -4891,7 +4982,7 @@
         if (s->haux) hipStreamSynchronize(s->haux->stream);
         s->beta_deferred = false; s->beta_pending = false; s->prep_pending = false; s->z_filled_iter = 0;
         const double* d = ck[k % NS];
-        for (const Part& pt : parts()) {
+        for (const Part& pt : parts(true)) {
             if (hipMemcpyAsync(pt.p, d, pt.cnt * sizeof(double), hipMemcpyDeviceToDevice, st) != hipSuccess) return fail_hip("rollback");
             d += even(pt.cnt);
         }
diff --git a/gpirt_amd/csrc/stages.hip b/gpirt_amd/csrc/stages.hip
--- a/gpirt_amd/csrc/stages.hip
+++ b/gpirt_amd/csrc/stages.hip
@@ -338,7 +338,7 @@
     return __hiloint2double(hi, lo);
 }
 
-template <int EPT>
+template <int EPT, bool PK>
 __global__ __launch_bounds__(256) void draw_beta_reg_kernel(BetaArgs a)
 {
     static_assert(EPT <= 32, "one bit per row in the masks");
@@ -352,15 +352,21 @@
     const uint32_t item = a.item0 + (uint32_t)j;
     double F[EPT], T[EPT];
     uint32_t live = 0, neg = 0;
+    if (PK) {
+        const uint2 w = reinterpret_cast<const uint2*>(a.ypk)[j * 256 + t];
+        live = w.x; neg = w.y;
+    }
 #pragma unroll
     for (int e = 0; e < EPT; ++e) {
         const int i = t + 256 * e;
         const int ic = i < n ? i : n - 1;
-        const double yy = yj[ic];
         F[e] = fj[ic];
         T[e] = th[ic];
-        live |= (uint32_t)(i < n && yy == yy) << e;
-        neg |= (uint32_t)(yy < 0.0) << e;
+        if (!PK) {
+            const double yy = yj[ic];
+            live |= (uint32_t)(i < n && yy == yy) << e;
+            neg |= (uint32_t)(yy < 0.0) << e;
+        }
         if ((e & 7) == 7) __builtin_amdgcn_sched_barrier(0);
     }
     double cv[2] = { a.beta[0 + 2 * j], a.beta[1 + 2 * j] };
@@ -416,6 +422,7 @@
         have_kept = full;
     }
     if (t == 0) { a.beta[0 + 2 * j] = cv[0]; a.beta[1 + 2 * j] = cv[1]; }
+    if (a.beta_mu && t == 0) { a.beta_mu[0 + 2 * j] = cv[0]; a.beta_mu[1 + 2 * j] = cv[1]; }
     if (a.mu) {
         double* __restrict__ mj = a.mu + j * a.n;
         int t2 = t;
@@ -424,6 +431,16 @@
         for (int e = 0; e < EPT; ++e) {
             const int i = t2 + 256 * e;
             if (i < n) mj[i] = cv[0] + T[e] * cv[1];
+            if ((e & 7) == 7) __builtin_amdgcn_sched_barrier(0);
+        }
+    }
+    if (PK && a.theta_mu && j == 0) {
+        int t2 = t;
+        asm volatile("" : "+v"(t2));
+#pragma unroll
+        for (int e = 0; e < EPT; ++e) {
+            const int i = t2 + 256 * e;
+            if (i < n) a.theta_mu[i] = T[e];
             if ((e & 7) == 7) __builtin_amdgcn_sched_barrier(0);
         }
     }
@@ -438,6 +455,24 @@
 #undef DB_SCREEN_PASS
 #undef DB_FULL_PASS
 
+__global__ __launch_bounds__(256) void beta_pack_kernel(const double* __restrict__ y, int64_t n, uint32_t* __restrict__ out)
+{
+    const int64_t j = blockIdx.x;
+    const int t = threadIdx.x;
+    const double* __restrict__ yj = y + j * n;
+    uint32_t live = 0, neg = 0;
+#pragma unroll 8
+    for (int e = 0; e < 32; ++e) {
+        const int64_t i = t + 256 * e;
+        if (i < n) {
+            const double yy = yj[i];
+            live |= (uint32_t)(yy == yy) << e;
+            neg |= (uint32_t)(yy < 0.0) << e;
+        }
+    }
+    reinterpret_cast<uint2*>(out)[j * 256 + t] = make_uint2(live, neg);
+}
+
 __global__ void linear_mean_kernel(const double* __restrict__ x, int64_t n, const double* __restrict__ beta,
                                    int64_t m, double* __restrict__ mu)
 {
@@ -537,10 +572,25 @@
 {
     if (a.m <= 0) return 0;
     const bool reg = a.screen == 1 && a.U == nullptr && a.n >= 1 && a.n <= 256 * 32;
-    if (reg && a.n <= 256 * 8) hipLaunchKernelGGL(draw_beta_reg_kernel<8>, dim3((unsigned)a.m), dim3(256), 0, stream, a);
-    else if (reg && a.n <= 256 * 16) hipLaunchKernelGGL(draw_beta_reg_kernel<16>, dim3((unsigned)a.m), dim3(256), 0, stream, a);
-    else if (reg) hipLaunchKernelGGL(draw_beta_reg_kernel<32>, dim3((unsigned)a.m), dim3(256), 0, stream, a);
+    if ((a.ypk || a.beta_mu || a.theta_mu) && !reg) { set_error("launch_draw_beta: packed y and beta_mu go with the register kernel (item RNG, 1 <= n <= 8192)"); return GPIRT_E_ARG; }
+    if (reg && a.ypk) {
+        if (a.n <= 256 * 8) hipLaunchKernelGGL((draw_beta_reg_kernel<8, true>), dim3((unsigned)a.m), dim3(256), 0, stream, a);
+        else if (a.n <= 256 * 16) hipLaunchKernelGGL((draw_beta_reg_kernel<16, true>), dim3((unsigned)a.m), dim3(256), 0, stream, a);
+        else hipLaunchKernelGGL((draw_beta_reg_kernel<32, true>), dim3((unsigned)a.m), dim3(256), 0, stream, a);
+    }
+    else if (reg && a.n <= 256 * 8) hipLaunchKernelGGL((draw_beta_reg_kernel<8, false>), dim3((unsigned)a.m), dim3(256), 0, stream, a);
+    else if (reg && a.n <= 256 * 16) hipLaunchKernelGGL((draw_beta_reg_kernel<16, false>), dim3((unsigned)a.m), dim3(256), 0, stream, a);
+    else if (reg) hipLaunchKernelGGL((draw_beta_reg_kernel<32, false>), dim3((unsigned)a.m), dim3(256), 0, stream, a);
     else hipLaunchKernelGGL(draw_beta_kernel, dim3((unsigned)a.m), dim3(256), 0, stream, a);
+    GP_HIP(hipGetLastError());
+    return 0;
+}
+
+int launch_beta_pack(hipStream_t stream, const double* y, int64_t n, int64_t m, uint32_t* out)
+{
+    if (m <= 0) return 0;
+    if (n < 1 || n > 256 * 32) { set_error("launch_beta_pack: n = %lld, the register kernel takes 1 <= n <= 8192", (long long)n); return GPIRT_E_ARG; }
+    hipLaunchKernelGGL(beta_pack_kernel, dim3((unsigned)m), dim3(256), 0, stream, y, n, out);
     GP_HIP(hipGetLastError());
     return 0;
 }
diff --git a/gpirt_amd/ops.py b/gpirt_amd/ops.py
--- a/gpirt_amd/ops.py
+++ b/gpirt_amd/ops.py
@@ -289,6 +289,22 @@
                                              n, m, seed, it, _p(path)))
         return beta, path.t()
 
+    def beta_pack(self, y):
+        n, m = y.shape
+        out = torch.zeros((m, 256, 2), dtype=torch.int32, device=y.device)
+        check(self.lib.gpirt_beta_pack(self._h, _p(y), n, m, _p(out)))
+        return out
+
+    def draw_beta_packed(self, beta, theta, y, f, pm, ps, step, seed: int, it: int, mu: bool = True):
+        n, m = y.shape
+        ypk = torch.zeros((m, 256, 2), dtype=torch.int32, device=y.device)
+        path = torch.full((m, 2), -1, dtype=torch.int32, device=y.device)
+        mu_out = colmajor(n, m, y.device) if mu else None
+        beta_mu = colmajor(2, m, y.device)
+        check(self.lib.gpirt_draw_beta_packed(self._h, _p(beta), _p(theta), _p(y), _p(f), _p(pm), _p(ps), _p(step),
+                                              n, m, seed, it, _p(ypk), _p(mu_out) if mu else C.c_void_p(0), _p(beta_mu), _p(path)))
+        return beta, path.t(), mu_out, beta_mu
+
     def prof_enable(self, on: bool):
         check(self.lib.gpirt_prof_enable(self._h, int(on)))
 
diff --git a/gpirt_amd/sampler.py b/gpirt_amd/sampler.py
--- a/gpirt_amd/sampler.py
+++ b/gpirt_amd/sampler.py
@@ -577,6 +577,12 @@
         return r.value
 
     @property
+    def beta_pack_draws(self) -> int:
+        r = C.c_int64()
+        check(self.lib.gpirt_sampler_beta_pack_draws(self._s, C.byref(r)))
+        return r.value
+
+    @property
     def ess_pack_draws(self) -> int:
         r = C.c_int64()
         check(self.lib.gpirt_sampler_ess_pack_draws(self._s, C.byref(r)))
diff --git a/include/gpirt_hip.h b/include/gpirt_hip.h
--- a/include/gpirt_hip.h
+++ b/include/gpirt_hip.h
@@ -124,6 +124,13 @@
                         const double* d_theta, const double* d_beta, int64_t n, int64_t m, uint64_t seed,
                         uint32_t iter, int* d_k_out);
 int gpirt_sampler_ess_pack_draws(gpirt_sampler_t s, int64_t* draws);
+
+int gpirt_beta_pack(gpirt_handle_t h, const double* d_y, int64_t n, int64_t m, uint32_t* d_ypk);
+int gpirt_draw_beta_packed(gpirt_handle_t h, double* d_beta, const double* d_theta, const double* d_y,
+                           const double* d_f, const double* d_pm, const double* d_ps, const double* d_step,
+                           int64_t n, int64_t m, uint64_t seed, uint32_t iter, uint32_t* d_ypk, double* d_mu,
+                           double* d_beta_mu, int* d_path);
+int gpirt_sampler_beta_pack_draws(gpirt_sampler_t s, int64_t* draws);
 
 int gpirt_draw_fstar(gpirt_handle_t h, const double* d_f, const double* d_theta, const double* d_L,
                      int64_t ldl, const double* d_mu_star, int64_t n, int64_t m, uint64_t seed,
```
